# bertoldi-collab/DifFlexMM

Hardware: AMD Instinct MI355X
Metric: timesteps*rigid-units/s (forward + adjoint) (higher is better)
Workload: dtype f64

## Files before the change

difflexmm_amd/csrc/dfx_persist.h:

```cpp
#pragma once
#include "dfx_persist_api.h"

namespace {
using namespace dfx_persist;

typedef unsigned p_u4 __attribute__((ext_vector_type(4)));

__device__ __forceinline__ bool is_poison(double x) { return (unsigned)__double2hiint(x) == kPoisonWord; }

__device__ __forceinline__ void ring_load(const double* place, u32 byte_off, double (&r)[4]) {
  p_u4 c0, c1;
  asm volatile("global_load_dwordx4 %0, %2, %3 sc1\n\tglobal_load_dwordx4 %1, %2, %3 offset:16 sc1\n\ts_waitcnt vmcnt(0)"
               : "=&v"(c0), "=&v"(c1) : "v"(byte_off), "s"(place) : "memory");
  r[0] = __hiloint2double(c0.y, c0.x); r[1] = __hiloint2double(c0.w, c0.z);
  r[2] = __hiloint2double(c1.y, c1.x); r[3] = __hiloint2double(c1.w, c1.z);
}
__device__ __forceinline__ void ring_store(double* place, u32 byte_off, double a, double b) {
  p_u4 x;
  x.x = __double2loint(a); x.y = __double2hiint(a); x.z = __double2loint(b); x.w = __double2hiint(b);
  asm volatile("global_store_dwordx4 %0, %1, %2 sc1\n\ts_nop 1" ::"v"(byte_off), "v"(x), "s"(place) : "memory");
}
__device__ __forceinline__ void ring_poison(double* place, u32 byte_off) {
  p_u4 x; x.x = x.y = x.z = x.w = kPoisonWord;
  asm volatile("global_store_dwordx4 %0, %1, %2 sc1\n\ts_nop 1" ::"v"(byte_off), "v"(x), "s"(place) : "memory");
}

__global__ __launch_bounds__(kThreads) void k_ring_poison(double* ring, int batch, int n_blocks, int m0, int width , int places) {
  const int m = blockIdx.y + m0;
  const int tid = blockIdx.x * kThreads + threadIdx.x;
  if (tid >= n_blocks * width) return;
  const unsigned long long p = ~0ull;
  for (int pl = 0; pl < places; ++pl)
    reinterpret_cast<unsigned long long*>(ring)[((size_t)pl * batch + m) * ((size_t)n_blocks * width) + tid] = p;
}

struct LigRes {
  double rox, roy, rpx, rpy, lx, ly, l0, il0, ks, ksh, kr, sgn;
  double am, ac, kc, phi1, phi2, kap_safe, phi_min;
  int info, pslot;
};
template <int CONTACT>
__device__ __forceinline__ void load_lig_res(const DevCtx& c, const MemberBases& B, int slot, LigRes& g) {
  g.info = ldg<int>(c.slot_info, (u32)slot * 4);
  g.pslot = g.info < 0 ? slot : (g.info >> 1);
  g.sgn = (g.info & 1) ? 1.0 : -1.0;
  const double2 ro = ldg<double2>(B.p_r, (u32)slot * 16), rp = ldg<double2>(B.p_r, (u32)g.pslot * 16);
  g.rox = ro.x; g.roy = ro.y; g.rpx = rp.x; g.rpy = rp.y;
  if (c.l_dict_on) {
    const u32 li = (u32)ldg<uint8_t>(B.p_lidx, (u32)slot);
    const double2 lv = ldg<double2>(B.l_dict, li * 32), ln = ldg<double2>(B.l_dict, li * 32 + 16);
    g.lx = lv.x; g.ly = lv.y; g.l0 = ln.x; g.il0 = ln.y;
  } else {
    const double2 lv = ldg<double2>(B.p_l, (u32)slot * 16);
    g.lx = lv.x; g.ly = lv.y;
    g.l0 = g.info < 0 ? 1.0 : sqrt(lv.x * lv.x + lv.y * lv.y);
    g.il0 = 1.0 / g.l0;
  }
  if (c.k_uniform) { g.ks = B.cst[3]; g.ksh = B.cst[4]; g.kr = B.cst[5]; }
  else { g.ks = ldg<double>(B.p_k, (u32)slot * 32); g.ksh = ldg<double>(B.p_k, (u32)slot * 32 + 8); g.kr = ldg<double>(B.p_k, (u32)slot * 32 + 16); }
  g.am = g.ac = g.kc = g.phi1 = g.phi2 = g.kap_safe = g.phi_min = 0.0;
  if (CONTACT == 1) {
    g.am = B.cst[0]; g.ac = B.cst[1]; g.kc = B.cst[2]; g.kap_safe = B.cst[9]; g.phi_min = B.cst[10];
    const double2 ph = ldg<double2>(B.p_phi, (u32)slot * 16);
    g.phi1 = ph.x; g.phi2 = ph.y;
  }
}
__device__ __forceinline__ bool ring_wait(const double* place, u32 byte_off, double (&r)[4], int t_ord, int* give_up, int limit) {
  for (int spins = 0;;) {
    ring_load(place, byte_off, r);
    const bool ok = !(is_poison(r[0]) || is_poison(r[1]) || is_poison(r[2]) || is_poison(r[3]));
    if (__all(ok)) return true;
    if (++spins > limit) { *give_up = 1 + t_ord; return false; }
    __builtin_amdgcn_s_sleep(1);
  }
}

#ifdef DFX_PERSIST_TIMING
__device__ __forceinline__ unsigned long long tick() {
  unsigned long long t;
  asm volatile("s_waitcnt vmcnt(0) lgkmcnt(0)\n\ts_memtime %0\n\ts_waitcnt lgkmcnt(0)" : "=s"(t)::"memory");
  return t;
}
#if DFX_PERSIST_TIMING == 2
#define DFX_TICK(k) if ((k) < 4) { unsigned long long t_; asm volatile("s_memtime %0\n\ts_waitcnt lgkmcnt(0)" : "=s"(t_)::"memory"); acc_t[k] += (unsigned)(t_ - t_prev); t_prev = t_; }
#else
#define DFX_TICK(k) { const unsigned long long t_ = tick(); acc_t[k] += (unsigned)(t_ - t_prev); t_prev = t_; }
#endif
#else
#define DFX_TICK(k)
#endif

__device__ __forceinline__ bool persist_wave(const PersistArgs& pa, int& ml, int& w) {
  const int wv = (int)(threadIdx.x >> 6);
  if (pa.xcd_wg > 0) {
    const int xcd = (int)(blockIdx.x & 7), pos = (int)(blockIdx.x >> 3);
    const int mi = pos / pa.xcd_wg, j = pos - mi * pa.xcd_wg;
    ml = __builtin_amdgcn_readfirstlane(mi * 8 + xcd);
    w = __builtin_amdgcn_readfirstlane(j * (kPersistThreads / 64) + wv);
    return ml < pa.nm && w < pa.waves_per_member;
  }
  const int wave = __builtin_amdgcn_readfirstlane((int)(blockIdx.x * (kPersistThreads / 64)) + wv);
  if (wave >= pa.waves_per_member * pa.nm) return false;
  ml = wave / pa.waves_per_member;
  w = wave - ml * pa.waves_per_member;
  return true;
}

template <int NPB>
__device__ __forceinline__ LanePos wave_lane_pos(int w, int n_blocks) {
  LanePos p;
  const int gtid = w * 64 + (int)(threadIdx.x & 63);
  if (NPB == 4) { p.slot = gtid; p.b = gtid >> 2; p.k = gtid & 3; p.valid = p.b < n_blocks; return p; }
  const int j = gtid & 15;
  const int tri = min((j * 11) >> 5, 4);
  p.k = j - 3 * tri;
  p.b = (gtid >> 4) * 5 + tri;
  p.valid = p.b < n_blocks;
  p.slot = p.b * 4 + p.k;
  return p;
}

#ifndef DFX_PERSIST_OCC
#define DFX_PERSIST_OCC
#endif
template <int MODEL, int CONTACT, int NPB>
__global__ __launch_bounds__(kPersistThreads) DFX_PERSIST_OCC void k_fwd_persist(DevCtx c, PersistCoef pc, PersistArgs pa) {
  int ml, w;
  if (!persist_wave(pa, ml, w)) return;
  const int m = c.m0 + ml;
  const LanePos lp = wave_lane_pos<NPB>(w, c.n_blocks);
  if (!lp.valid) return;
  const int slot = lp.slot, b = lp.b, k = lp.k, kd = k < 3 ? k : 2;
  const u32 nd = (u32)c.n_blocks * 3;
  const int s = c.s;
  const Seg sg = *c.cur;
  const MemberBases B = member_bases(c, m);
  LigRes g;
  load_lig_res<CONTACT>(c, B, slot, g);
  const int info = g.info, pslot = g.pslot;
  const int dof = b * 3 + kd;
  const u32 o_dof = (u32)dof * 8, o_rec = ((u32)b * kPos + kd) * 8, o_chunk = ((u32)b * kPos + 2 * (k & 1)) * 8;
  const double damp = c.damping_uniform ? B.cst[6 + kd] : ldg<double>(c.damping + (size_t)((u32)m * nd), o_dof);
  const double invm = ldg<double>(c.inv_m + (size_t)((u32)m * nd), o_dof);
  const int sidx = ldg<int>(c.block_special, (u32)b * 4);
  const bool constrained = k < 3 && sidx >= 0 && ((c.special[sidx >= 0 ? sidx : 0].con_mask >> k) & 1);
  double tf_coef[DFX_MAX_FNS];
#pragma unroll
  for (int f = 0; f < DFX_MAX_FNS; ++f)
    tf_coef[f] = (k < 3 && sidx >= 0 && f < c.n_fns) ? (constrained ? c.special[sidx].con_coef[k][f] : c.special[sidx].load_coef[k][f]) : 0.0;
  const bool recs = c.rps > 1;
  const long long n0 = sg.base_step;
  double qn, vn;
  BlockRec<double> o;
  {
    const double* P0 = pos_in(c, m, recs ? -1 : 0, n0);
    const double* V0 = vel_in(c, m, recs ? -1 : 0, n0);
    const double2 a0 = ldg<double2>(P0, (u32)b * kPos * 8), a1 = ldg<double2>(P0, (u32)b * kPos * 8 + 16);
    o.x = a0.x; o.y = a0.y; o.th = a1.x; o.sh = a1.y;
    qn = ldg<double>(P0, o_rec);
    vn = ldg<double>(V0, o_dof);
  }
  double al[kPersistStages];
#pragma unroll
  for (int l = 0; l < kPersistStages; ++l) al[l] = 0.0;
  const size_t ring_stride = (size_t)c.batch * c.n_blocks * kPos;
  const u32 r_own = ((u32)m * (u32)c.n_blocks + (u32)b) * (kPos * 8) + 16u * (u32)(k & 1);
  const u32 r_par = ((u32)m * (u32)c.n_blocks + (u32)(pslot >> 2)) * (kPos * 8);
  if (k < 2) ring_store(pa.ring, r_own, k == 0 ? o.x : o.th, k == 0 ? o.y : o.sh);
  const int total = pa.n_steps * s;
  int t_ord = 0;
  double v_i = vn;
#ifdef DFX_PERSIST_TIMING
  unsigned acc_t[6] = {0, 0, 0, 0, 0, 0};
  unsigned long long t_prev = tick();
  const unsigned long long t_first = t_prev, w_first = wall_clock64();
#endif
  for (int j = 0; j < pa.n_steps; ++j) {
    const long long n = n0 + j;
    double h = sg.h;
    if (c.t_steps) { const double* ts = steps_of(c, m); h = ts[n + 1] - ts[n]; }
    double* Am = c.AD ? c.AD + (size_t)m * c.ad_stride + (size_t)n * ((u32)(s - 1) * nd) : nullptr;
#pragma unroll 1
    for (int i = 0; i < s; ++i) {
      {
        o.ch = half_cos(o.th, o.sh);
        double sv = 0.0, sq = 0.0, fload = 0.0;
#pragma unroll
        for (int l = 0; l < kPersistStages - 1; ++l) {
          const double a_l = l < i ? al[l] : 0.0;
          sv += pc.cv[i][l] * a_l;
          sq += pc.cq[i][l] * a_l;
        }
        double tv0[DFX_MAX_FNS], tv1[DFX_MAX_FNS];
#pragma unroll
        for (int f = 0; f < DFX_MAX_FNS; ++f) { tv0[f] = 0.0; tv1[f] = 0.0; }
        if (k < 3 && sidx >= 0) {
          const double* ft = fn_tab_row(c, m, j, constrained ? i + 1 : i);
          const u32 z = lane_zero();
#pragma unroll
          for (int f = 0; f < DFX_MAX_FNS; ++f)
            if (f < c.n_fns) { tv0[f] = fn_tab_get(ft, f, 0, z); if (constrained) tv1[f] = fn_tab_get(ft, f, 1, z); }
        }
        DFX_TICK(0)
        const double* place = pa.ring + (size_t)(t_ord % kPRing) * ring_stride;
        double pr[4];
        if (!ring_wait(place, r_par, pr, t_ord, pa.give_up, pa.spin_limit)) return;
        DFX_TICK(1)
        if (k < 2 && t_ord + kPAhead <= total) ring_poison(pa.ring + (size_t)((t_ord + kPAhead) % kPRing) * ring_stride, r_own);
        BlockRec<double> p;
        p.x = pr[0]; p.y = pr[1]; p.th = pr[2]; p.sh = pr[3];
        p.ch = half_cos(p.th, p.sh);
        double q_pre = 0.0, v_pre = 0.0;
#pragma unroll
        for (int f = 0; f < DFX_MAX_FNS; ++f) {
          if (constrained) { q_pre += tf_coef[f] * tv0[f]; v_pre += tf_coef[f] * tv1[f]; }
          else fload += tf_coef[f] * tv0[f];
        }
        double fx = 0.0, fy = 0.0, fth = 0.0;
        if (info >= 0) {
          BondGrad<double> bg;
          bond_grad<MODEL, double>(o, p, g.rox, g.roy, g.rpx, g.rpy, g.lx, g.ly, g.l0, g.il0, g.ks, g.ksh, g.kr, g.sgn, bg);
          fx = bg.fx; fy = bg.fy; fth = bg.fth;
          if (CONTACT == 1) {
            const bool far = !(fabs(o.th - p.th) <= g.kap_safe);
            ContactGrad<double> cg;
            contact_grad<double>(g.sgn * (o.th - p.th), far ? g.phi1 : g.phi_min, far ? g.phi2 : g.phi_min, g.am, g.ac, g.kc, cg);
            fth += g.sgn * cg.dkap;
          }
        }
        DFX_TICK(2)
        const double dE = blk_reduce3<NPB>(fx, fy, fth, k);
        double qnext = 0.0, vnext = 0.0;
        if (k < 3) {
          const double a = constrained ? 0.0 : (fload - dE - damp * v_i) * invm;
          if (Am && i < s - 1) stg<double>(Am + (size_t)i * nd, o_dof, a);
          sv += pc.cv[i][i] * a;
          sq += pc.cq[i][i] * a;
#pragma unroll
          for (int l = 0; l < kPersistStages; ++l) al[l] = l == i ? a : al[l];
          qnext = qn + h * (pc.c[i + 1] * vn + h * sq);
          vnext = vn + h * sv;
          if (constrained) { qnext = q_pre; vnext = v_pre; }
        }
        DFX_TICK(3)
        const double y1 = blk_bcast<NPB, 1>(qnext, k), th2 = blk_bcast<NPB, 2>(qnext, k), x0 = blk_bcast<NPB, 0>(qnext, k);
        double sn, cs;
        fast_sincos(0.5 * th2, &sn, &cs);
        o.x = x0; o.y = y1; o.th = th2; o.sh = sn;
        ++t_ord;
        DFX_TICK(4)
        const bool last = i == s - 1;
        if (k < 2) ring_store(pa.ring + (size_t)(t_ord % kPRing) * ring_stride, r_own, k == 0 ? x0 : th2, k == 0 ? y1 : sn);
        if (k < 3) {
          const double2 chunk = k == 0 ? make_double2(x0, y1) : make_double2(th2, sn);
          if (recs || (last && c.traj)) {
            double* tr = recs ? traj_rec(c, m, -2 - i, n) : traj_rec(c, m, -1, n + 1);
            if (k < 2) stg<double2>(tr, o_chunk, chunk);
            stg<double>(tr + (size_t)c.n_blocks * kPos, o_dof, vnext);
          }
          if (last && !recs && j == pa.n_steps - 1) {
            if (k < 2) stg<double2>(c.POS + (size_t)((u32)m * (u32)c.nbuf * (u32)c.n_blocks * kPos), o_chunk, chunk);
            stg<double>(c.VEL + (size_t)((u32)m * (u32)c.nbuf * nd), o_dof, vnext);
          }
        }
        v_i = vnext;
        if (last) { qn = qnext; vn = vnext; }
        DFX_TICK(5)
      }
    }
  }
#ifdef DFX_PERSIST_TIMING
  if (pa.dbg && (threadIdx.x & 63) == 0) {
    unsigned* d = pa.dbg + (size_t)(blockIdx.x * 4 + (threadIdx.x >> 6)) * 8;
    for (int q = 0; q < 6; ++q) d[q] = acc_t[q];
    d[6] = (unsigned)(tick() - t_first); d[7] = (unsigned)total;
  }
  if (blockIdx.x == 0 && threadIdx.x == 0) {
    for (int q = 0; q < 6; ++q) pa.give_up[1 + q] = (int)acc_t[q];
    pa.give_up[7] = (int)(tick() - t_first);
    pa.give_up[8] = (int)(wall_clock64() - w_first);
    pa.give_up[9] = total;
  }
#endif
}



template <int MODEL, int CONTACT, int NPB, int DENSE>
__device__ __forceinline__ void adj_persist_body(const DevCtx& c, const PersistAdjCoef& pc, const PersistArgs& pa, const DenseCtx& dn) {
  int ml, w;
  if (!persist_wave(pa, ml, w)) return;
  const int m = c.m0 + ml;
  const LanePos lp = wave_lane_pos<NPB>(w, c.n_blocks);
  if (!lp.valid) return;
  const int slot = lp.slot, b = lp.b, k = lp.k, kd = k < 3 ? k : 2;
  const u32 nd = (u32)c.n_blocks * 3, nd6 = (u32)c.n_blocks * 6;
  const int s = c.s;
  const Seg sg = *c.cur;
  long long n_m = 0;
  int j_top = pa.n_steps - 1;
  if constexpr (DENSE) {
    n_m = dn.n_acc[m];
    if (n_m - sg.base_step < (long long)j_top) j_top = (int)(n_m - sg.base_step);
    if (j_top < 0) return;
  }
  const MemberBases B = member_bases(c, m);
  LigRes g;
  load_lig_res<CONTACT>(c, B, slot, g);
  const int info = g.info, pslot = g.pslot;
  const int dof = b * 3 + kd;
  const u32 o_dof = (u32)dof * 8, o_b6 = ((u32)b * 6 + 2 * kd) * 8;
  const double damp = c.damping_uniform ? B.cst[6 + kd] : ldg<double>(c.damping + (size_t)((u32)m * nd), o_dof);
  const double invm = ldg<double>(c.inv_m + (size_t)((u32)m * nd), o_dof);
  const int sidx = ldg<int>(c.block_special, (u32)b * 4);
  const bool constrained = k < 3 && sidx >= 0 && ((c.special[sidx >= 0 ? sidx : 0].con_mask >> k) & 1);
  double tf_coef[DFX_MAX_FNS];
#pragma unroll
  for (int f = 0; f < DFX_MAX_FNS; ++f)
    tf_coef[f] = (k < 3 && sidx >= 0 && f < c.n_fns) ? (constrained ? c.special[sidx].con_coef[k][f] : c.special[sidx].load_coef[k][f]) : 0.0;
  double* LAMm = c.LAM + (size_t)((u32)m * nd6);
  const u32 ms = (u32)m * (u32)c.n_slots;
  double* grm = c.g_r + (size_t)(ms * 2);
  double* gpm = c.g_phi + (size_t)ms;
  double* bmm = c.blk_m + (size_t)((u32)m * nd);
  double* bcm = c.blk_c ? c.blk_c + (size_t)((u32)m * nd) : nullptr;
  __shared__ double2 s_yb[kPersistStages - 1][kPersistThreads];
  __shared__ double2 s_racc[kPersistThreads];
  __shared__ double s_acc[3][kPersistThreads];
  __shared__ double2 s_lam[kPersistThreads];
  const int tid = (int)threadIdx.x;
  s_racc[tid] = ldg<double2>(grm, (u32)slot * 16);
  s_lam[tid] = ldg<double2>(LAMm, o_b6);
  s_acc[0][tid] = CONTACT == 1 ? ldg<double>(gpm, (u32)slot * 8) : 0.0;
  s_acc[1][tid] = ldg<double>(bmm, o_dof);
  s_acc[2][tid] = bcm ? ldg<double>(bcm, o_dof) : 0.0;
  bool phi_any = false;
  const size_t ring_stride = (size_t)c.batch * c.n_blocks * kPos;
  const u32 r_own = ((u32)m * (u32)c.n_blocks + (u32)b) * (kPos * 8) + 16u * (u32)(k & 1);
  const u32 r_par = ((u32)m * (u32)c.n_blocks + (u32)(pslot >> 2)) * (kPos * 8);
  const int total = DENSE ? (j_top + 1) * s - ((sg.base_step + j_top == n_m) ? s - 1 : 0) : pa.n_steps * s;
  int t_ord = 0;
#ifdef DFX_PERSIST_TIMING
  unsigned acc_t[6] = {0, 0, 0, 0, 0, 0};
  unsigned long long t_prev = tick();
  const unsigned long long t_first = t_prev;
#endif
  for (int j = j_top; j >= 0; --j) {
    const long long n = sg.base_step + j;
    double h = sg.h, h_before = (sg.j0 + j) == 0 ? sg.h_prev : sg.h;
    if (c.t_steps) { const double* ts = steps_of(c, m); h = ts[n + 1] - ts[n]; h_before = n > 0 ? ts[n] - ts[n - 1] : 0.0; }
#pragma unroll 1
    for (int i = (DENSE && n == n_m) ? 0 : s - 1; i >= 0; --i) {
      const int win = (int)((n * s + i) & 1);
      const double* POSin = traj_rec(c, m, -1 - i, n);
      const double2 o0 = ldg<double2>(POSin, (u32)b * (kPos * 8)), o1 = ldg<double2>(POSin, (u32)b * (kPos * 8) + 16);
      const double2 q0 = ldg<double2>(POSin, (u32)(pslot >> 2) * (kPos * 8)), q1 = ldg<double2>(POSin, (u32)(pslot >> 2) * (kPos * 8) + 16);
      const double v_i = ldg<double>(POSin + (size_t)c.n_blocks * kPos, o_dof);
      double sq = 0.0, sv = 0.0, sqc = 0.0, svc = 0.0;
#pragma unroll
      for (int jj = 1; jj < kPersistStages; ++jj) {
        const bool on = jj > i && jj < s && !(DENSE && n == n_m);
        const double2 y = on ? s_yb[jj - 1][tid] : make_double2(0.0, 0.0);
        const double cf = i > 0 ? pc.col[i][jj] : 1.0;
        sq += cf * y.x;
        sv += cf * y.y;
        sqc += pc.cur[i][jj] * y.x;
        svc += pc.cur[i][jj] * y.y;
      }
      double tv0[DFX_MAX_FNS];
#pragma unroll
      for (int f = 0; f < DFX_MAX_FNS; ++f) tv0[f] = 0.0;
      if (k < 3 && sidx >= 0 && !constrained) {
        const double* ft = fn_tab_row(c, m, j, i);
        const u32 z = lane_zero();
#pragma unroll
        for (int f = 0; f < DFX_MAX_FNS; ++f) if (f < c.n_fns) tv0[f] = fn_tab_get(ft, f, 0, z);
      }
      const double col_s = pc.col[i][s], cur_s = pc.cur[i][s], col_i = pc.col[i][i];
      const double2 lam = s_lam[tid];
      const double lq = lam.x, lv = lam.y;
      double w_d = (h * (cur_s * lv + svc)) * invm;
      double e_own_q = 0.0, e_nxt_v = 0.0, gs_q = 0.0, gs_v = 0.0;
      if constexpr (DENSE) {
        if (!constrained) {
          const int* op = dn.out_ptr + (size_t)m * dn.stride;
          const int lo = op[n], hi = op[n + 1], plo = n > 0 ? op[n - 1] : lo;
          const double* dwm = dn.dw + (size_t)m * dn.n_out * 8;
          const u32 o_g = ((u32)b * 6 + kd) * 8;
          double e_own_v = 0.0;
          for (int kk = lo; kk < hi; ++kk) {
            const double* Gk = c.G + ((size_t)kk * c.batch + m) * (size_t)nd6;
            const double gq = ldg<double>(Gk, o_g), gv = ldg<double>(Gk, o_g + 24);
            const double* wt = dwm + (size_t)kk * 8;
            e_own_q += wt[i] * gq; e_own_v += wt[i] * gv;
            if (i > 0) e_nxt_v += wt[i - 1] * gv;
            else { gs_q += gq; gs_v += gv; }
          }
          e_own_q *= h; e_own_v *= h; e_nxt_v *= h;
          if (i <= 1) {
            double e6q = 0.0, e6v = 0.0, e5v = 0.0;
            for (int kk = plo; kk < lo; ++kk) {
              const double* Gk = c.G + ((size_t)kk * c.batch + m) * (size_t)nd6;
              const double gq = ldg<double>(Gk, o_g), gv = ldg<double>(Gk, o_g + 24);
              const double* wt = dwm + (size_t)kk * 8;
              e6q += wt[6] * gq; e6v += wt[6] * gv;
              e5v += wt[s - 1] * gv;
            }
            if (i == 0) { e_own_q += h_before * e6q; e_own_v += h_before * e6v; e_nxt_v = h_before * e5v; }
            else e_nxt_v += h_before * e6v;
          }
          if (i == 0 && n == 0)
            for (int kk = 0; kk < lo; ++kk) {
              const double* Gk = c.G + ((size_t)kk * c.batch + m) * (size_t)nd6;
              gs_q += ldg<double>(Gk, o_g); gs_v += ldg<double>(Gk, o_g + 24);
            }
          w_d += e_own_v * invm;
        }
      }
      const double wox = blk_bcast<NPB, 0>(w_d, k), woy = blk_bcast<NPB, 1>(w_d, k), woth = blk_bcast<NPB, 2>(w_d, k);
      double wp[4];
      DFX_TICK(0)
      if (t_ord == 0) {
        const double* Win = c.W + (size_t)(((u32)m * 2 + (u32)win) * nd);
        const u32 pb = (u32)(pslot >> 2) * 24;
        const double2 wxy = ldg<double2>(Win, pb);
        wp[0] = wxy.x; wp[1] = wxy.y; wp[2] = ldg<double>(Win, pb + 16);
      } else if (!ring_wait(pa.ring + (size_t)(t_ord % kPRing) * ring_stride, r_par, wp, t_ord, pa.give_up, pa.spin_limit)) return;
      DFX_TICK(1)
      if (k < 2 && t_ord + kPAhead < total) ring_poison(pa.ring + (size_t)((t_ord + kPAhead) % kPRing) * ring_stride, r_own);
      BlockRec<double> o, p;
      o.x = o0.x; o.y = o0.y; o.th = o1.x; o.sh = o1.y; o.ch = half_cos(o.th, o.sh);
      p.x = q0.x; p.y = q0.y; p.th = q1.x; p.sh = q1.y; p.ch = half_cos(p.th, p.sh);
      double hx = 0.0, hy = 0.0, hth = 0.0, ex = 0.0, ey = 0.0, eth = 0.0, d_rx = 0.0, d_ry = 0.0, d_phi = 0.0;
      if (info >= 0) {
        BondHvp hv;
        bond_hvp<MODEL>(o, p, wox, woy, woth, wp[0], wp[1], wp[2], g.rox, g.roy, g.rpx, g.rpy, g.lx, g.ly, g.l0, g.il0, g.ks, g.ksh, g.kr, g.sgn, hv);
        hx = hv.hx; hy = hv.hy; hth = hv.hth;
        ex = hv.fx; ey = hv.fy; eth = hv.fth;
        d_rx = hv.rx; d_ry = hv.ry;
        if (CONTACT == 1) {
          const bool far = !(fabs(o.th - p.th) <= g.kap_safe);
          double dk, dke, p1e, p2e;
          contact_hvp(g.sgn * (o.th - p.th), g.sgn * (woth - wp[2]), far ? g.phi1 : g.phi_min, far ? g.phi2 : g.phi_min, g.am, g.ac, g.kc, dk, dke, p1e, p2e);
          hth += g.sgn * dke;
          eth += g.sgn * dk;
          d_phi = (info & 1) ? p2e : p1e;
        }
        const double2 r_old = s_racc[tid];
        s_racc[tid] = make_double2(r_old.x - d_rx, r_old.y - d_ry);
      }
      if (CONTACT == 1 && d_phi != 0.0) { s_acc[0][tid] -= d_phi; phi_any = true; }
      DFX_TICK(2)
      const double hw = blk_reduce3<NPB>(hx, hy, hth, k);
      const double dE = blk_reduce3<NPB>(ex, ey, eth, k);
      double w_next = 0.0;
      if (k < 3) {
        double fload = 0.0;
#pragma unroll
        for (int f = 0; f < DFX_MAX_FNS; ++f) if (!constrained) fload += tf_coef[f] * tv0[f];
        if (c.fn_g && sidx >= 0) {
          const double* ft = fn_tab_row(c, m, j, i);
#pragma unroll
          for (int f = 0; f < DFX_MAX_FNS; ++f) {
            const double coef = f < c.n_fns ? (constrained ? -hw * tf_coef[f] : w_d * tf_coef[f]) : 0.0;
            if (coef != 0.0) {
              const u32 z = lane_zero();
              double* q = c.fn_g + (((size_t)m * c.n_special + sidx) * DFX_MAX_FNS + f) * DFX_FN_PARAMS;
              for (int kk = 0; kk < DFX_FN_PARAMS; ++kk) acc_add(q + kk, coef * fn_tab_get(ft, f, 2 + kk, z));
            }
          }
        }
        const double a_i = constrained ? 0.0 : (fload - dE - damp * v_i) * invm;
        double kq_in = h * (cur_s * lq + sqc);
        if constexpr (DENSE) kq_in += e_own_q;
        double ybq = 0.0, ybv = 0.0;
        if (!constrained) {
          ybq = -hw;
          ybv = kq_in - damp * w_d;
          s_acc[1][tid] -= w_d * a_i;
          s_acc[2][tid] -= w_d * v_i;
        }
        if (i > 0) s_yb[i - 1][tid] = make_double2(ybq, ybv);
        double kv;
        if (i > 0) {
          kv = h * (col_s * lv + col_i * ybv + sv);
        } else {
          double nlq = lq + (ybq + sq), nlv = lv + (ybv + sv);
          if constexpr (DENSE) { nlq += gs_q; nlv += gs_v; }
          const bool first = !DENSE && (sg.j0 + j) == 0;
          if (first && c.G && !constrained) {
            const double* G = c.G + ((size_t)sg.interval * c.batch + m) * (size_t)nd6;
            nlq += G[b * 6 + k]; nlv += G[b * 6 + 3 + k];
          }
          if (constrained) { nlq = 0.0; nlv = 0.0; }
          s_lam[tid] = make_double2(nlq, nlv);
          kv = h_before * col_s * nlv;
        }
        if constexpr (DENSE) kv += e_nxt_v;
        w_next = constrained ? 0.0 : kv * invm;
      }
      DFX_TICK(3)
      ++t_ord;
      if (t_ord < total) {
        const double w1 = blk_bcast<NPB, 1>(w_next, k), w2 = blk_bcast<NPB, 2>(w_next, k);
        if (k < 2) ring_store(pa.ring + (size_t)(t_ord % kPRing) * ring_stride, r_own, k == 0 ? w_next : w2, k == 0 ? w1 : 0.0);
      } else if (k < 3) {
        stg<double>(c.W + (size_t)(((u32)m * 2 + (u32)(win ^ 1)) * nd), o_dof, w_next);
      }
    }
  }
#ifdef DFX_PERSIST_TIMING
  if (pa.dbg && (threadIdx.x & 63) == 0) {
    unsigned* d = pa.dbg + (size_t)(blockIdx.x * 4 + (threadIdx.x >> 6)) * 8;
    for (int q = 0; q < 6; ++q) d[q] = acc_t[q];
    d[6] = (unsigned)(tick() - t_first); d[7] = (unsigned)total;
  }
#endif
  if (info >= 0) stg<double2>(grm, (u32)slot * 16, s_racc[tid]);
  if (CONTACT == 1 && phi_any) { stg<double>(gpm, (u32)slot * 8, s_acc[0][tid]); c.touch[0] = 1; }
  if (k < 3) {
    stg<double2>(LAMm, o_b6, s_lam[tid]);
    if (!constrained) { stg<double>(bmm, o_dof, s_acc[1][tid]); if (bcm) stg<double>(bcm, o_dof, s_acc[2][tid]); }
  }
}

template <int MODEL, int CONTACT, int NPB>
__global__ __launch_bounds__(kPersistThreads) __attribute__((amdgpu_waves_per_eu(3))) void k_adj_persist(DevCtx c, PersistAdjCoef pc, PersistArgs pa) {
  adj_persist_body<MODEL, CONTACT, NPB, 0>(c, pc, pa, DenseCtx{});
}

}
```

difflexmm_amd/csrc/dfx_persist_api.h:

```cpp
#pragma once
#include <hip/hip_runtime.h>

namespace dfx_persist {

constexpr int kPRing = 8;
constexpr int kPAhead = 4;
constexpr int kPersistThreads = 256;
constexpr unsigned kPoisonWord = 0xFFFFFFFFu;
constexpr int kPersistStages = 6;
constexpr int kSpinLimit = 1 << 23;
static_assert(kPAhead >= 2 && kPRing >= kPAhead + 1, "hand-off ring: re-poison at least two ordinals ahead, ring longer than the look-ahead");

struct PersistCoef {
  double cv[kPersistStages][kPersistStages];
  double cq[kPersistStages][kPersistStages];
  double c[kPersistStages + 1];
};
struct PersistArgs {
  double* ring;
  int* give_up;
  int n_steps, nm, waves_per_member;
  int spin_limit;
  int xcd_wg;
#ifdef DFX_PERSIST_TIMING
  unsigned* dbg;
#endif
};


struct PersistAdjCoef {
  double col[kPersistStages][kPersistStages + 1];
  double cur[kPersistStages][kPersistStages + 1];
  double c[kPersistStages];
};

const void* fwd_kernel(int model, int contact, int npb);
const void* adj_kernel(int model, int contact, int npb);
const void* adaptive_fwd_kernel(int model, int contact);
const void* adj_dense_kernel(int model, int contact, int npb);
void launch_ring_poison(hipStream_t st, double* ring, int batch, int n_blocks, int m0, int nm, int width);

}
```

difflexmm_amd/csrc/dfx_persist_dense.h:

```cpp
#pragma once
#include "dfx_persist.h"
#include "dfx_dense.h"

template <int CTRL> __device__ __forceinline__ double dpp_row_mov(double v) {
  int lo = __double2loint(v), hi = __double2hiint(v);
  lo = __builtin_amdgcn_update_dpp(lo, lo, CTRL, 0xf, 0xf, false);
  hi = __builtin_amdgcn_update_dpp(hi, hi, CTRL, 0xf, 0xf, false);
  return __hiloint2double(hi, lo);
}
__device__ __forceinline__ double lanes_plus_32(double v) {
  const unsigned lo = (unsigned)__double2loint(v), hi = (unsigned)__double2hiint(v);
  const auto a = __builtin_amdgcn_permlane32_swap(lo, lo, false, false);
  const auto b = __builtin_amdgcn_permlane32_swap(hi, hi, false, false);
  return __hiloint2double((int)b[1], (int)a[1]);
}
__device__ __forceinline__ double lanes_plus_16(double v) {
  const unsigned lo = (unsigned)__double2loint(v), hi = (unsigned)__double2hiint(v);
  const auto a = __builtin_amdgcn_permlane16_swap(lo, lo, false, false);
  const auto b = __builtin_amdgcn_permlane16_swap(hi, hi, false, false);
  return __hiloint2double((int)b[1], (int)a[1]);
}
__device__ __forceinline__ double wave_sum_lane0(double v) {
  v += lanes_plus_32(v);
  v += lanes_plus_16(v);
  v += dpp_row_mov<0x108>(v);
  v += dpp_row_mov<0x104>(v);
  v += dpp_row_mov<0x102>(v);
  v += dpp_row_mov<0x101>(v);
  return v;
}
__device__ __forceinline__ double lane_value(double v, int lane_uniform) {
  return __hiloint2double(__builtin_amdgcn_readlane(__double2hiint(v), lane_uniform), __builtin_amdgcn_readlane(__double2loint(v), lane_uniform));
}

#ifndef DFX_DENSE_OCC
#define DFX_DENSE_OCC __attribute__((amdgpu_waves_per_eu(3)))
#endif
namespace {

__device__ __forceinline__ double err_load(const double* p) {
  double v;
  asm volatile("global_load_dwordx2 %0, %1, off sc1\n\ts_waitcnt vmcnt(0)" : "=&v"(v) : "v"(p) : "memory");
  return v;
}
__device__ __forceinline__ void err_store(double* p, double v) {
  asm volatile("global_store_dwordx2 %0, %1, off sc1\n\ts_nop 1" ::"v"(p), "v"(v) : "memory");
}

template <int MODEL, int CONTACT>
__global__ __launch_bounds__(kPersistThreads) void k_adaptive_fwd_loop(DevCtx c, AdaptLoopCoef pc, PersistArgs pa, AdaptLoopArgs aa) {
  int ml, w;
  if (!persist_wave(pa, ml, w)) return;
  const int W = pa.waves_per_member;
  const int m = c.m0 + ml;
  Clock ck = c.clock[m];
  if (ck.state) return;
  LanePos lp = wave_lane_pos<4>(w, c.n_blocks);
  const bool valid = lp.valid;
  if (!valid) { lp.b = c.n_blocks - 1; lp.k = (int)(threadIdx.x & 3); lp.slot = lp.b * 4 + lp.k; }
  const int slot = lp.slot, b = lp.b, k = lp.k, kd = k < 3 ? k : 2;
  const int lane = (int)(threadIdx.x & 63);
  const u32 nd = (u32)c.n_blocks * 3;
  const MemberBases B = member_bases(c, m);
  LigRes g;
  load_lig_res<CONTACT>(c, B, slot, g);
  const int info = g.info, pslot = g.pslot;
  const int dof = b * 3 + kd;
  const u32 o_dof = (u32)dof * 8, o_rec = ((u32)b * kPos + kd) * 8, o_chunk = ((u32)b * kPos + 2 * (k & 1)) * 8;
  const double damp = c.damping_uniform ? B.cst[6 + kd] : ldg<double>(c.damping + (size_t)((u32)m * nd), o_dof);
  const double invm = ldg<double>(c.inv_m + (size_t)((u32)m * nd), o_dof);
  const int sidx = ldg<int>(c.block_special, (u32)b * 4);
  const bool constrained = k < 3 && sidx >= 0 && ((c.special[sidx >= 0 ? sidx : 0].con_mask >> k) & 1);
  const bool dof_lane = valid && k < 3;
  const bool keep = aa.keep != 0;
  double tf_coef[DFX_MAX_FNS];
#pragma unroll
  for (int f = 0; f < DFX_MAX_FNS; ++f)
    tf_coef[f] = (valid && k < 3 && sidx >= 0 && f < c.n_fns) ? (constrained ? c.special[sidx].con_coef[k][f] : c.special[sidx].load_coef[k][f]) : 0.0;
  double* Am = c.A + (size_t)((u32)m * (u32)(c.s + 1) * nd);
  long long n_acc = ck.accepted;
  double qn, vn;
  BlockRec<double> o;
  {
    const double* P0 = pos_in(c, m, keep ? -1 : 0, n_acc);
    const double* V0 = vel_in(c, m, keep ? -1 : 0, n_acc);
    const double2 a0 = ldg<double2>(P0, (u32)b * kPos * 8), a1 = ldg<double2>(P0, (u32)b * kPos * 8 + 16);
    o.x = a0.x; o.y = a0.y; o.th = a1.x; o.sh = a1.y;
    qn = ldg<double>(P0, o_rec);
    vn = ldg<double>(V0, o_dof);
  }
  double al[7];
  al[0] = ldg<double>(Am, o_dof);
#pragma unroll
  for (int l = 1; l < 7; ++l) al[l] = 0.0;
  const size_t ring_stride = (size_t)c.batch * c.n_blocks * kPos;
  const u32 r_own = ((u32)m * (u32)c.n_blocks + (u32)b) * (kPos * 8) + 16u * (u32)(k & 1);
  const u32 r_par = ((u32)m * (u32)c.n_blocks + (u32)(pslot >> 2)) * (kPos * 8);
  const size_t err_stride = (size_t)c.batch * W;
  double* err_m = aa.err + (size_t)m * W;
  const double* ts_out = c.ts_dev;
  const int Tn = aa.n_timepoints;
  double t = ck.t, h = ck.h;
  double t_out_next = ck.out_idx < Tn ? ts_out[ck.out_idx] : 1.7976931348623157e308;
  int t_ord = 0;
  long long attempt = 0;
  for (; attempt < pa.n_steps; ++attempt) {
    if (keep && n_acc + 3 > aa.cap) break;
    double fg[DFX_MAX_FNS], fgt[DFX_MAX_FNS];
    const bool need_fn = c.n_fns > 0 && __any(sidx >= 0);
    if (need_fn) {
      const int jj = min(lane & 7, 6);
      const double cj = jj == 0 ? pc.c[0] : (jj == 1 ? pc.c[1] : (jj == 2 ? pc.c[2] : (jj == 3 ? pc.c[3] : (jj == 4 ? pc.c[4] : (jj == 5 ? pc.c[5] : pc.c[6])))));
      double gp[kMaxFnParams];
#pragma unroll
      for (int f = 0; f < DFX_MAX_FNS; ++f) {
        fg[f] = 0.0; fgt[f] = 0.0;
        if (f < c.n_fns) eval_time_fn(c.fns[(u32)m * DFX_MAX_FNS + f], t + cj * h, fg[f], fgt[f], gp);
      }
    }
    auto prescribed = [&](int j, double& q, double& v) {
      if (!need_fn) return;
      double sq_ = 0.0, sv_ = 0.0;
#pragma unroll
      for (int f = 0; f < DFX_MAX_FNS; ++f) {
        const double gj = lane_value(fg[f], j), gtj = lane_value(fgt[f], j);
        if (constrained && f < c.n_fns) { sq_ += tf_coef[f] * gj; sv_ += tf_coef[f] * gtj; }
      }
      if (constrained) { q = sq_; v = sv_; }
    };
    auto load_at = [&](int j) -> double {
      double fl = 0.0;
      if (!need_fn) return fl;
#pragma unroll
      for (int f = 0; f < DFX_MAX_FNS; ++f) {
        const double gj = lane_value(fg[f], j);
        if (k < 3 && sidx >= 0 && !constrained && f < c.n_fns) fl += tf_coef[f] * gj;
      }
      return fl;
    };
    double v_i;
    {
      double qx = qn + h * pc.a[1][0] * vn, vx = vn + h * pc.a[1][0] * al[0];
      prescribed(1, qx, vx);
      v_i = vx;
      const double y1 = blk_bcast<4, 1>(qx, k), th2 = blk_bcast<4, 2>(qx, k), x0 = blk_bcast<4, 0>(qx, k);
      double sn, cs;
      fast_sincos(0.5 * th2, &sn, &cs);
      o.x = x0; o.y = y1; o.th = th2; o.sh = sn;
      if (valid && k < 2) ring_store(pa.ring + (size_t)(t_ord % kPRing) * ring_stride, r_own, k == 0 ? x0 : th2, k == 0 ? y1 : sn);
      if (keep && dof_lane) {
        double* tr = traj_rec(c, m, -2, n_acc);
        if (k < 2) stg<double2>(tr, o_chunk, k == 0 ? make_double2(x0, y1) : make_double2(th2, sn));
        stg<double>(tr + (size_t)c.n_blocks * kPos, o_dof, vx);
      }
    }
    double q1 = 0.0, v1 = 0.0, r2 = 0.0;
#pragma unroll 1
    for (int i = 1; i <= 6; ++i) {
      o.ch = half_cos(o.th, o.sh);
      double sv = 0.0, sq = 0.0, fload = 0.0;
#pragma unroll
      for (int l = 0; l < 6; ++l) {
        const double a_l = l < i ? al[l] : 0.0;
        sv += (i < 6 ? pc.a[i + 1][l] : pc.e[l]) * a_l;
        sq += (i < 6 ? pc.aa[i + 1][l] : pc.ee[l]) * a_l;
      }
      fload = load_at(i);
      double pr[4];
      if (!ring_wait(pa.ring + (size_t)(t_ord % kPRing) * ring_stride, r_par, pr, t_ord, pa.give_up, pa.spin_limit)) return;
      if (valid && k < 2) ring_poison(pa.ring + (size_t)((t_ord + kPAhead) % kPRing) * ring_stride, r_own);
      BlockRec<double> p;
      p.x = pr[0]; p.y = pr[1]; p.th = pr[2]; p.sh = pr[3];
      p.ch = half_cos(p.th, p.sh);
      double fx = 0.0, fy = 0.0, fth = 0.0;
      if (info >= 0) {
        BondGrad<double> bg;
        bond_grad<MODEL, double>(o, p, g.rox, g.roy, g.rpx, g.rpy, g.lx, g.ly, g.l0, g.il0, g.ks, g.ksh, g.kr, g.sgn, bg);
        fx = bg.fx; fy = bg.fy; fth = bg.fth;
        if (CONTACT == 1) {
          const bool far = !(fabs(o.th - p.th) <= g.kap_safe);
          ContactGrad<double> cg;
          contact_grad<double>(g.sgn * (o.th - p.th), far ? g.phi1 : g.phi_min, far ? g.phi2 : g.phi_min, g.am, g.ac, g.kc, cg);
          fth += g.sgn * cg.dkap;
        }
      }
      const double dE = blk_reduce3<4>(fx, fy, fth, k);
      const double a = constrained ? 0.0 : (fload - dE - damp * v_i) * invm;
      ++t_ord;
      if (i < 6) {
        sv += pc.a[i + 1][i] * a;
        sq += pc.aa[i + 1][i] * a;
#pragma unroll
        for (int l = 1; l < 7; ++l) al[l] = l == i ? a : al[l];
        double qx = qn + h * (pc.c[i + 1] * vn + h * sq), vx = vn + h * sv;
        prescribed(i + 1, qx, vx);
        const double y1 = blk_bcast<4, 1>(qx, k), th2 = blk_bcast<4, 2>(qx, k), x0 = blk_bcast<4, 0>(qx, k);
        double sn, cs;
        fast_sincos(0.5 * th2, &sn, &cs);
        o.x = x0; o.y = y1; o.th = th2; o.sh = sn;
        if (valid && k < 2) ring_store(pa.ring + (size_t)(t_ord % kPRing) * ring_stride, r_own, k == 0 ? x0 : th2, k == 0 ? y1 : sn);
        if (keep && dof_lane) {
          double* tr = traj_rec(c, m, -2 - i, n_acc);
          if (k < 2) stg<double2>(tr, o_chunk, k == 0 ? make_double2(x0, y1) : make_double2(th2, sn));
          stg<double>(tr + (size_t)c.n_blocks * kPos, o_dof, vx);
        }
        v_i = vx;
        if (i == 5) { q1 = qx; v1 = vx; }
      } else {
        al[6] = a;
        sv += pc.e[6] * a;
        sq += pc.ee[6] * a;
        if (dof_lane && !constrained) {
          const double eq = h * h * sq, ev = h * sv;
          const double tq = c.atol + c.rtol * fmax(fabs(qn), fabs(q1)), tv = c.atol + c.rtol * fmax(fabs(vn), fabs(v1));
          r2 = (eq / tq) * (eq / tq) + (ev / tv) * (ev / tv);
        }
      }
    }
    r2 = wave_sum_lane0(r2);
    double* slot_now = err_m + (size_t)(attempt % 3) * err_stride;
    if (lane == 0) err_store(slot_now + w, r2);
    double acc_a = 0.0, acc_b = 0.0;
    for (int r = 0; r * 64 < W; ++r) {
      const int idx = lane + 64 * r;
      double v = 0.0;
      if (idx < W) {
        for (int spins = 0;;) {
          v = err_load(slot_now + idx);
          if (!is_poison(v)) break;
          if (++spins > pa.spin_limit) { *pa.give_up = -1 - (int)(attempt & 0xffff); return; }
          __builtin_amdgcn_s_sleep(1);
        }
      }
      if (r & 1) acc_b += v; else acc_a += v;
    }
    if (lane == 0) err_store(err_m + (size_t)((attempt + 2) % 3) * err_stride + w, __hiloint2double((int)kPoisonWord, (int)kPoisonWord));
    double red = acc_a + acc_b;
    red = lane_value(wave_sum_lane0(red), 0);
    const double ratio = sqrt(red / aa.two_n_free);
    ck.attempts++;
    if (!(ratio == ratio)) { ck.state = 2; break; }
    const double h_new = dopri_next_step(h, ratio);
    if (ratio <= 1.0) {
      const double t_new = t + h;
      const int out_lo = ck.out_idx;
      int out_hi = out_lo;
      if (t_out_next <= t_new) {
        while (out_hi < Tn && ts_out[out_hi] <= t_new) ++out_hi;
        t_out_next = out_hi < Tn ? ts_out[out_hi] : 1.7976931348623157e308;
      }
      if (dof_lane && out_hi > out_lo) {
        double sm = pc.cm[0] * al[0] + pc.cm[6] * al[6], sma = pc.cma[0] * al[0] + pc.cma[6] * al[6];
#pragma unroll
        for (int l = 1; l < 6; ++l) { sm += pc.cm[l] * al[l]; sma += pc.cma[l] * al[l]; }
        const double qmid = qn + h * (0.5 * vn + h * sma), vmid = vn + h * sm;
        for (int kk = out_lo; kk < out_hi; ++kk) {
          const double tk = ts_out[kk];
          const double r = (tk - t) / (t_new - t);
          double oq = dopri_dense(qn, q1, qmid, vn, v1, h, r), ov = dopri_dense(vn, v1, vmid, al[0], al[6], h, r);
          if (constrained) { const TimeVals tv = constrained_value(c, m, c.special[sidx], k, tk); oq = tv.g; ov = tv.gt; }
          double* f = c.fields_dev + ((size_t)m * Tn + kk) * c.n_blocks * 6;
          stg<double>(f, o_dof, oq);
          stg<double>(f + nd, o_dof, ov);
        }
      }
      if (w == 0 && lane == 0) {
        if (c.acc_times && n_acc + 1 <= c.acc_cap) c.acc_times[(size_t)m * c.acc_cap + n_acc] = t_new;
        if (c.step_counts && Tn > 1) c.step_counts[(size_t)m * (Tn - 1) + min(max(out_lo - 1, 0), Tn - 2)]++;
        if (aa.ar.t_steps) {
          double* ts = aa.ar.t_steps + (size_t)m * aa.ar.stride;
          int* op = aa.ar.out_ptr + (size_t)m * aa.ar.stride;
          ts[n_acc + 1] = t_new; ts[n_acc + 2] = t_new;
          op[n_acc] = out_lo; op[n_acc + 1] = out_hi; op[n_acc + 2] = out_hi;
          for (int kk = out_lo; kk < out_hi; ++kk) aa.ar.theta[(size_t)m * Tn + kk] = (ts_out[kk] - t) / (t_new - t);
        }
      }
      ck.t_last = t; ck.h_acc = h; ck.out_lo = out_lo; ck.out_hi = out_hi; ck.out_idx = out_hi; ck.accepted++;
      t = t_new; ++n_acc;
      qn = q1; vn = v1; al[0] = al[6];
      if (out_hi >= Tn) { ck.state = 1; ck.h = h_new; break; }
    }
    ck.accept = ratio <= 1.0;
    h = h_new;
    if (!(h > 0.0)) { ck.state = 3; break; }
  }
  ck.t = t; if (ck.state != 1) ck.h = h;
  if (w == 0 && lane == 0) c.clock[m] = ck;
  const double y1 = blk_bcast<4, 1>(qn, k), th2 = blk_bcast<4, 2>(qn, k), x0 = blk_bcast<4, 0>(qn, k);
  double sn, cs;
  fast_sincos(0.5 * th2, &sn, &cs);
  if (dof_lane) {
    stg<double>(Am, o_dof, al[0]);
    if (!keep) {
      if (k < 2) stg<double2>(c.POS + (size_t)((u32)m * (u32)c.nbuf * (u32)c.n_blocks * kPos), o_chunk, k == 0 ? make_double2(x0, y1) : make_double2(th2, sn));
      stg<double>(c.VEL + (size_t)((u32)m * (u32)c.nbuf * nd), o_dof, vn);
    }
  }
}

template <int MODEL, int CONTACT, int NPB>
__global__ __launch_bounds__(kPersistThreads) DFX_DENSE_OCC void k_adj_dense_loop(DevCtx c, PersistAdjCoef pc, PersistArgs pa,
                                                                                                           DenseCtx dn) {
  adj_persist_body<MODEL, CONTACT, NPB, 1>(c, pc, pa, dn);
}

}
```

difflexmm_amd/csrc/engine_launch.hip:

```cpp
#include "dfx_engine.h"
#include <climits>

using namespace dfx_persist;

void drop_graphs(dfx_handle* h) {
  for (auto& kv : h->graphs) (void)hipGraphExecDestroy(kv.second);
  h->graphs.clear();
  h->graph_ctx_valid = false;
  if (h->adaptive_exec) { (void)hipGraphExecDestroy(h->adaptive_exec); h->adaptive_exec = nullptr; }
}

DevCtx make_ctx(dfx_handle* h) {
  const Plan& pl = h->pl;
  DevCtx c;
  memset(&c, 0, sizeof(c));
  c.n_blocks = pl.n_blocks; c.n_slots = pl.n_slots; c.n_fns = pl.n_fns; c.batch = pl.batch; c.s = pl.tab.s;
#ifdef DFX_ABLATE
  { const char* a = getenv("DFX_ABLATE"); c.ablate = a ? atoi(a) : 0; }
#endif
  c.n_wg = (pl.n_slots + kThreads - 1) / kThreads;
  c.n_wg3 = (pl.n_blocks + (kThreads / 16) * 5 - 1) / ((kThreads / 16) * 5);
  for (int k = 0; k < 4; ++k) c.pred[k] = pl.pred_delta[k];
  c.nbuf = 2 * pl.tab.s;
  c.n_special = pl.n_special; c.k_uniform = h->pp.k_uniform ? 1 : 0; c.n_timepoints = (int)h->ts.size();
  c.slot_info = h->d_slot_info.p; c.block_special = h->d_block_special.p; c.special = h->d_special.p;
  c.n_ovf = pl.n_ovf;
  if (pl.n_ovf) { c.ovf_ptr = h->d_ovf_ptr.p; c.ovf_info = h->d_ovf_info.p; c.ovf_p = h->d_ovf_p.p; c.ovf_g = h->d_ovf_g.p; }
  c.p_lidx = h->d_l_idx.p; c.l_dict = h->d_l_dict.p; c.l_dict_on = h->pp.l_dict_ok ? 1 : 0; c.damping_uniform = h->pp.damping_uniform ? 1 : 0;
  { const char* e = getenv("DFX_DICT_LDS"); c.l_dict_lds = (h->pp.l_dict_ok && h->pp.n_dict_max <= kDictLds && !(e && e[0] == '0')) ? 1 : 0; }
  c.p_r = h->d_p_r.p; c.p_l = h->d_p_l.p; c.p_k = h->d_p_k.p; c.p_phi = h->d_p_phi.p; c.cst = h->d_cst.p;
  c.inv_m = h->d_inv_m.p; c.damping = h->d_damping.p; c.fns = h->d_fns.p;
  c.p_c = h->d_p_c.p; c.g_c = h->d_g_c.p; c.n_npb = pl.n_npb;
  c.cur = h->d_cur.p;
  c.fn_tab = nullptr;
  c.clock = h->adaptive ? h->d_clock.p : nullptr;
  c.err_partial = h->d_err_partial.p; c.ts_dev = h->d_ts.p; c.fields_dev = h->d_fields.p;
  c.step_counts = h->adaptive ? h->d_step_counts.p : nullptr;
  c.acc_times = h->adaptive ? h->d_acc_times.p : nullptr; c.acc_cap = kAccCap;
  c.t_steps = (!h->adaptive && !h->t_steps.empty()) ? h->d_tsteps.p : nullptr;
  c.ts_stride = c.t_steps ? h->ts_stride : 0;
  c.rtol = h->rtol; c.atol = h->atol;
  c.traj = h->have_traj ? h->ck->traj.p : nullptr;
  c.rps = (h->have_traj && (h->records || h->segments)) ? pl.tab.s : 1;
  c.AD = (h->have_traj && h->dense && !h->records && !h->segments) ? h->ck->AD.p : nullptr;
  c.ad_stride = pl.batch ? (long long)(h->ck->AD.n / pl.batch) : 0;
  c.POS = h->d_POS.p; c.VEL = h->d_VEL.p; c.A = h->d_A.p;
  c.YB = h->d_YB.p; c.LAM = h->d_LAM.p; c.W = h->d_W.p; c.KQ = h->d_KQ.p; c.G = h->d_G.p;
  c.g_r = h->d_g_r.p; c.g_phi = h->d_g_phi.p; c.g_b = (h->want_bond_grads || pl.n_ovf) ? h->d_g_b.p : nullptr;
  c.touch = h->d_touch.p;
  c.lam_pairs = (c.g_b || c.AD) ? 0 : 1;
  c.blk_m = h->d_blk_m.p; c.blk_c = h->want_damping_grads ? h->d_blk_c.p : nullptr;
  c.fn_g = h->want_fn_grads ? h->d_fn_g.p : nullptr;
  return c;
}

dim3 slot_grid(const dfx_handle* h) { return dim3((h->pl.n_slots + kThreads - 1) / kThreads, h->pl.batch); }
dim3 slot_grid(const dfx_handle* h, const Group& g) { return dim3((h->pl.n_slots + kThreads - 1) / kThreads, g.nm); }
DevCtx group_ctx(const dfx_handle* h, const DevCtx& c, int gi) {
  DevCtx cg = c;
  cg.m0 = h->groups[gi].m0;
  cg.cur = h->d_cur.p + gi;
  return cg;
}

StageCoef stage_coef(const Tableau& T, int i) {
  StageCoef sc;
  memset(&sc, 0, sizeof(sc));
  const int r = i + 1;
  for (int l = 0; l <= i; ++l) { sc.cv[l] = T.a[r][l]; sc.cq[l] = T.aa[r][l]; }
  sc.c_i = T.c[i];
  sc.c_next = T.c[r];
  return sc;
}
AdjCoef adj_coef(const Tableau& T, int i) {
  AdjCoef ac;
  memset(&ac, 0, sizeof(ac));
  if (i > 0) {
    for (int j = i; j < T.s; ++j) ac.col[j] = T.a[j][i - 1];
    ac.col[T.s] = T.a[T.s][i - 1];
  } else {
    ac.col[T.s] = T.a[T.s][T.s - 1];
  }
  for (int j = i + 1; j < T.s; ++j) ac.cur[j] = T.a[j][i];
  ac.cur[T.s] = T.a[T.s][i];
  ac.c_i = T.c[i];
  return ac;
}

#ifdef DFX_EXPERIMENTAL
#include "dfx_experimental_host.h"
#else
void setup_tiling(dfx_handle*) {}
void setup_lig(dfx_handle*) {}
int lig_pack(dfx_handle*) { return 0; }
void pair_plan(dfx_handle* h, const DevCtx&) { h->pair_fwd = h->pair_adj = false; }
bool lig_fwd_ok(const dfx_handle*, const DevCtx&, int) { return false; }
bool lig_adj_ok(const dfx_handle*, const DevCtx&, int, int) { return false; }
#endif
int pair_state_buf(const dfx_handle* h, long long n) {
#ifdef DFX_EXPERIMENTAL
  if (h->pair_fwd) return state_buf(n);
#endif
  (void)h; (void)n;
  return 0;
}

bool pack3(const dfx_handle* h) {
  const char* e = getenv("DFX_PACK3");
  return h->pl.n_npb == 3 && !h->adaptive && !(e && e[0] == '0');
}
static bool hot_shape(const DevCtx& c) {
  return c.k_uniform && c.l_dict_on && c.l_dict_lds && c.damping_uniform && !c.t_steps && !c.AD && !c.clock;
}
template <int MODEL, int CONTACT, int NPB>
static bool launch_fwd_hot(dfx_handle* h, const DevCtx& c, hipStream_t st, dim3 grid, int i, int j, int in_buf, int out_buf, int y_buf, int mode) {
  if constexpr ((MODEL == kNonlinear || MODEL == kLinearized) && CONTACT != 2) {
    if (!h->wt || !h->stage_builds || !hot_shape(c)) return false;
    const StageCoef scf = stage_coef(h->pl.tab, i);
    const bool recs = c.rps > 1 && in_buf == -1 - i && out_buf == -2 - i && y_buf == -1 && mode == 0;
#define DFX_FWD_I(I)                                                                                                              \
  case I:                                                                                                                         \
    if (recs)                                                                                                                     \
      hipLaunchKernelGGL((k_fwd_stage<MODEL, CONTACT, NPB, 1, 0, 1, I, 1>), grid, dim3(kThreads), 0, st, c, scf, i, j, in_buf, out_buf, \
                         y_buf, mode);                                                                                            \
    else                                                                                                                          \
      hipLaunchKernelGGL((k_fwd_stage<MODEL, CONTACT, NPB, 1, 0, 1, I, 0>), grid, dim3(kThreads), 0, st, c, scf, i, j, in_buf, out_buf, \
                         y_buf, mode);                                                                                            \
    return true;
    switch (i) { DFX_FWD_I(0) DFX_FWD_I(1) DFX_FWD_I(2) DFX_FWD_I(3) DFX_FWD_I(4) DFX_FWD_I(5) default: break; }
#undef DFX_FWD_I
  }
  return false;
}
namespace dfx_hot {
bool launch_adj_stage_build(int model, int contact, int npb, hipStream_t st, dim3 grid, const DevCtx& c, const AdjCoef& acf, int i, int j, int in_buf, int wbuf,
                            int local_only, const StageCoef& rc, int rb);
}
template <int MODEL, int CONTACT, int NPB>
static bool launch_adj_hot(dfx_handle* h, const DevCtx& c, hipStream_t st, dim3 grid, int i, int j, int in_buf, int wbuf, int local_only, const StageCoef& rc,
    int rb) {
  if constexpr ((MODEL == kNonlinear || MODEL == kLinearized) && CONTACT != 2) {
    if (!h->wt || !h->stage_builds || !(c.k_uniform && c.l_dict_on && c.l_dict_lds && c.damping_uniform && !c.t_steps)) return false;
    return dfx_hot::launch_adj_stage_build(MODEL, CONTACT, NPB, st, grid, c, adj_coef(h->pl.tab, i), i, j, in_buf, wbuf, local_only, rc, rb);
  }
  return false;
}
int kernel_build_code(const dfx_handle* h, const DevCtx& c, bool tile) {
  if (tile) return 1;
  const bool model_ok = (h->pl.model == kNonlinear || h->pl.model == kLinearized) && h->pl.contact != DFX_CONTACT_DISTANCE;
  const bool quad_or_packed = !h->pl.n_ovf && (h->pl.n_npb == 4 || pack3(h));
  return (model_ok && quad_or_packed && h->wt && h->stage_builds && c.fn_tab && hot_shape(c) && h->pl.tab.s <= 6) ? 2 : 0;
}
template <int MODEL, int CONTACT>
static void launch_fwd_t(dfx_handle* h, const DevCtx& c, hipStream_t st, dim3 grid, int i, int j, int in_buf, int out_buf, int y_buf, int mode) {
#ifdef DFX_EXPERIMENTAL
  if constexpr (CONTACT != 2) {
    if (lig_fwd_ok(h, c, mode)) {
      const dim3 tg(h->lig.n_wg, grid.y);
      hipLaunchKernelGGL((k_fwd_tile<MODEL, CONTACT>), tg, dim3(64 * kTileWaves), 0, st, c, h->lig, stage_coef(h->pl.tab, i), i, j, in_buf, out_buf,
                         y_buf, mode);
      return;
    }
  }
#endif
  if (h->pl.n_ovf) {
    if constexpr (CONTACT != 2)
      hipLaunchKernelGGL((k_fwd_stage<MODEL, CONTACT, 4, 0, 1>), grid, dim3(kThreads), 0, st, c, stage_coef(h->pl.tab, i), i, j, in_buf, out_buf, y_buf, mode);
    return;
  }
  const bool tab = c.fn_tab != nullptr && !c.clock;
  if (CONTACT != 2 && pack3(h) && !(mode & 2)) {
    if constexpr (CONTACT != 2) {
      if (tab && launch_fwd_hot<MODEL, CONTACT, 3>(h, c, st, dim3(c.n_wg3, grid.y), i, j, in_buf, out_buf, y_buf, mode)) return;
      if (tab) hipLaunchKernelGGL((k_fwd_stage<MODEL, CONTACT, 3, 1>), dim3(c.n_wg3, grid.y), dim3(kThreads), 0, st, c, stage_coef(h->pl.tab, i), i, j,
          in_buf, out_buf, y_buf, mode);
      else hipLaunchKernelGGL((k_fwd_stage<MODEL, CONTACT, 3, 0>), dim3(c.n_wg3, grid.y), dim3(kThreads), 0, st, c, stage_coef(h->pl.tab, i), i, j, in_buf,
          out_buf, y_buf, mode);
    }
    return;
  }
  if (tab && h->wt) {
    if (launch_fwd_hot<MODEL, CONTACT, 4>(h, c, st, grid, i, j, in_buf, out_buf, y_buf, mode)) return;
    hipLaunchKernelGGL((k_fwd_stage<MODEL, CONTACT, 4, 1, 0, 1>), grid, dim3(kThreads), 0, st, c, stage_coef(h->pl.tab, i), i, j, in_buf, out_buf, y_buf, mode);
  }
  else if (tab) hipLaunchKernelGGL((k_fwd_stage<MODEL, CONTACT, 4, 1>), grid, dim3(kThreads), 0, st, c, stage_coef(h->pl.tab, i), i, j, in_buf, out_buf,
      y_buf, mode);
  else hipLaunchKernelGGL((k_fwd_stage<MODEL, CONTACT, 4, 0>), grid, dim3(kThreads), 0, st, c, stage_coef(h->pl.tab, i), i, j, in_buf, out_buf, y_buf, mode);
}
void launch_fwd(dfx_handle* h, const DevCtx& c, hipStream_t st, dim3 grid, int i, int j, int in_buf, int out_buf, int y_buf, int mode) {
  const Plan& pl = h->pl;
#define DFX_FWD_CASE(M) case M: if (pl.contact == 2) launch_fwd_t<M, 2>(h, c, st, grid, i, j, in_buf, out_buf, y_buf, mode); \
    else if (pl.contact) launch_fwd_t<M, 1>(h, c, st, grid, i, j, in_buf, out_buf, y_buf, mode); else launch_fwd_t<M, 0>(h, c, st, grid, i, j, in_buf, \
    out_buf, y_buf, mode); break;
  switch (pl.model) { DFX_FWD_CASE(kNonlinear) DFX_FWD_CASE(kLinearized) DFX_FWD_CASE(kSimpleSpring) DFX_FWD_CASE(kStretchTorsion) }
#undef DFX_FWD_CASE
  h->launches++;
}
void launch_fwd(dfx_handle* h, const DevCtx& c, int i, int j, int in_buf, int out_buf, int y_buf, int mode) {
  launch_fwd(h, c, h->stream, slot_grid(h), i, j, in_buf, out_buf, y_buf, mode);
}
template <int MODEL, int CONTACT>
static void launch_adj_t(dfx_handle* h, const DevCtx& c, hipStream_t st, dim3 grid, int i, int j, int in_buf, int wbuf, int local_only) {
  const int s = h->pl.tab.s;
  const int rb = (c.AD && !local_only) ? (i >= 2 ? i - 1 : (i == 0 ? s - 1 : 0)) : 0;
  const StageCoef rc = stage_coef(h->pl.tab, rb > 0 ? rb - 1 : 0);
#ifdef DFX_EXPERIMENTAL
  if constexpr (CONTACT != 2) {
    if (lig_adj_ok(h, c, wbuf, local_only)) {
      const dim3 tg(h->lig.n_wg, grid.y);
      hipLaunchKernelGGL((k_adj_tile<MODEL, CONTACT>), tg, dim3(64 * kTileWaves), 0, st, c, h->lig, adj_coef(h->pl.tab, i), i, j, in_buf);
      return;
    }
  }
#endif
  if (h->pl.n_ovf) {
    if constexpr (CONTACT != 2)
      hipLaunchKernelGGL((k_adj_stage<MODEL, CONTACT, 1, 1, 4, 0, 1>), grid, dim3(kThreads), 0, st, c, adj_coef(h->pl.tab, i), i, j, in_buf, wbuf, local_only,
          rc, rb);
  }
  else if (c.g_b) hipLaunchKernelGGL((k_adj_stage<MODEL, CONTACT, 1, 1>), grid, dim3(kThreads), 0, st, c, adj_coef(h->pl.tab, i), i, j, in_buf, wbuf,
      local_only, rc, rb);
  else if (c.AD) hipLaunchKernelGGL((k_adj_stage_rb<MODEL, CONTACT>), grid, dim3(kThreads), 0, st, c, adj_coef(h->pl.tab, i), i, j, in_buf, wbuf, local_only,
      rc, rb);
  else if (CONTACT != 2 && pack3(h)) {
    if constexpr (CONTACT != 2) {
      if (c.fn_tab && !local_only && launch_adj_hot<MODEL, CONTACT, 3>(h, c, st, dim3(c.n_wg3, grid.y), i, j, in_buf, wbuf, local_only, rc, rb)) return;
      if (c.fn_tab && !local_only) hipLaunchKernelGGL((k_adj_stage<MODEL, CONTACT, 0, 0, 3, 1>), dim3(c.n_wg3, grid.y), dim3(kThreads), 0, st, c,
          adj_coef(h->pl.tab, i), i, j, in_buf, wbuf, local_only, rc, rb);
      else hipLaunchKernelGGL((k_adj_stage<MODEL, CONTACT, 0, 0, 3, 0>), dim3(c.n_wg3, grid.y), dim3(kThreads), 0, st, c, adj_coef(h->pl.tab, i), i, j,
          in_buf, wbuf, local_only, rc, rb);
    }
  }
  else if (c.fn_tab && !local_only && h->wt) {
    if (launch_adj_hot<MODEL, CONTACT, 4>(h, c, st, grid, i, j, in_buf, wbuf, local_only, rc, rb)) return;
    hipLaunchKernelGGL((k_adj_stage<MODEL, CONTACT, 0, 0, 4, 1, 0, 1>), grid, dim3(kThreads), 0, st, c, adj_coef(h->pl.tab, i), i, j, in_buf, wbuf,
        local_only, rc, rb);
  }
  else if (c.fn_tab && !local_only) hipLaunchKernelGGL((k_adj_stage<MODEL, CONTACT, 0, 0, 4, 1>), grid, dim3(kThreads), 0, st, c, adj_coef(h->pl.tab, i), i,
      j, in_buf, wbuf, local_only, rc, rb);
  else hipLaunchKernelGGL((k_adj_stage<MODEL, CONTACT, 0, 0, 4, 0>), grid, dim3(kThreads), 0, st, c, adj_coef(h->pl.tab, i), i, j, in_buf, wbuf, local_only,
      rc, rb);
}
void launch_adj(dfx_handle* h, const DevCtx& c, hipStream_t st, dim3 grid, int i, int j, int in_buf, int wbuf, int local_only) {
  const Plan& pl = h->pl;
#define DFX_ADJ_CASE(M) case M: if (pl.contact == 2) launch_adj_t<M, 2>(h, c, st, grid, i, j, in_buf, wbuf, local_only); \
    else if (pl.contact) launch_adj_t<M, 1>(h, c, st, grid, i, j, in_buf, wbuf, local_only); else launch_adj_t<M, 0>(h, c, st, grid, i, j, in_buf, wbuf, \
    local_only); break;
  switch (pl.model) { DFX_ADJ_CASE(kNonlinear) DFX_ADJ_CASE(kLinearized) DFX_ADJ_CASE(kSimpleSpring) DFX_ADJ_CASE(kStretchTorsion) }
#undef DFX_ADJ_CASE
  h->launches++;
}
void launch_adj(dfx_handle* h, const DevCtx& c, int i, int j, int in_buf, int wbuf, int local_only) {
  launch_adj(h, c, h->stream, slot_grid(h), i, j, in_buf, wbuf, local_only);
}

static const int kPersistSlots = 64;
struct PersistInflight { hipEvent_t ev; hipStream_t st; int slots; };
static std::mutex g_persist_mu;
static std::vector<PersistInflight> g_persist_inflight[64];
static std::vector<hipEvent_t> g_persist_events[64];

static int persist_wg_slots(const void* fn) {
  static std::mutex mu;
  static std::map<const void*, int> cache;
  std::lock_guard<std::mutex> lk(mu);
  auto it = cache.find(fn);
  if (it != cache.end()) return it->second;
  hipFuncAttributes at;
  if (!fn || hipFuncGetAttributes(&at, fn) != hipSuccess) { (void)hipGetLastError(); return 0; }
  const int alloc = std::max(8, ((at.numRegs + 7) / 8) * 8);
  return cache[fn] = alloc > 512 ? 0 : alloc / 8;
}
static int persist_wg_per_cu(const void* fn) {
  static std::mutex mu;
  static std::map<const void*, int> cache;
  std::lock_guard<std::mutex> lk(mu);
  auto it = cache.find(fn);
  if (it != cache.end()) return it->second;
  int nb = 0;
  if (!fn || hipOccupancyMaxActiveBlocksPerMultiprocessor(&nb, fn, kPersistThreads, 0) != hipSuccess) { (void)hipGetLastError(); nb = 0; }
  return cache[fn] = nb;
}
bool persist_shape_ok(const dfx_handle* h) {
  const Plan& pl = h->pl;
  const char* e = getenv("DFX_PERSIST");
  if ((e && e[0] == '0') || h->persist_off) return false;
  return (pl.model == kNonlinear || pl.model == kLinearized) && pl.contact != DFX_CONTACT_DISTANCE && !pl.n_ovf && pl.tab.s <= kPersistStages &&
         (pl.n_npb == 3 || pl.n_npb == 4);
}
static int persist_waves_per_member(const dfx_handle* h, int npb) {
  return npb == 3 ? (h->pl.n_blocks + 19) / 20 : (h->pl.n_slots + 63) / 64;
}
static int persist_cap(const void* fn);
int persist_members_that_fit(dfx_handle* h, const void* fn, int npb) {
  if (!h->n_cu) { int v = 0; if (hipDeviceGetAttribute(&v, hipDeviceAttributeMultiprocessorCount, h->device) != hipSuccess || v <= 0) return 0; h->n_cu = v; }
  const int cap = persist_cap(fn);
  const long long wpm = persist_waves_per_member(h, npb);
  if (cap <= 0 || wpm <= 0) return 0;
  return (int)std::min<long long>(h->pl.batch, ((long long)cap * h->n_cu * 4) / wpm);
}
static int persist_cap(const void* fn) {
  const int wg_slots = persist_wg_slots(fn);
  int cap = wg_slots ? std::min(8, kPersistSlots / wg_slots) : 0;
  if (const int occ = persist_wg_per_cu(fn)) cap = std::min(cap, occ);
  if (const char* e = getenv("DFX_PERSIST_MAX_WG")) cap = std::min(cap, atoi(e));
  return cap;
}
static void persist_shape(const dfx_handle* h, int npb, int nm, int* grid, int* per_cu, const void* fn = nullptr, int* xcd_wg = nullptr) {
  const long long wpm = persist_waves_per_member(h, npb);
  if (xcd_wg) {
    *xcd_wg = 0;
    const char* e = getenv("DFX_PERSIST_XCD");
    const int wg = (int)((wpm + 3) / 4), cus = h->n_cu / 8, per_xcd = (nm + 7) / 8, cap = fn ? persist_cap(fn) : 0;
    if (!(e && e[0] == '0') && h->n_cu % 8 == 0 && wg <= cus && (long long)per_xcd * wg <= (long long)cap * cus) {
      *xcd_wg = wg;
      *grid = 8 * per_xcd * wg;
      *per_cu = std::max(1, (per_xcd * wg + cus - 1) / cus);
      return;
    }
  }
  const long long waves = (long long)nm * wpm;
  const long long g = (waves + 3) / 4;
  *grid = (int)g;
  *per_cu = (int)std::max<long long>(1, (g + h->n_cu - 1) / h->n_cu);
}
static int persist_max_chunks() {
  const char* e = getenv("DFX_PERSIST_CHUNKS");
  return e ? std::max(1, atoi(e)) : 2;
}
static int persist_adj_max_chunks() {
  const char* e = getenv("DFX_PERSIST_ADJ_CHUNKS");
  return e ? std::max(1, atoi(e)) : INT_MAX;
}
static int chunk_members(int nm, int n_chunks, int k) { return nm / n_chunks + (k < nm % n_chunks ? 1 : 0); }
static bool persist_common_ok(dfx_handle* h, const DevCtx& c, bool any_groups = false) {
  if (!persist_shape_ok(h) || h->adaptive || (h->groups.size() != 1 && !any_groups)) return false;
  if (h->pl.n_fns > 0 && !c.fn_tab) return false;
  h->persist_npb = (h->pl.n_npb == 3 && pack3(h)) ? 3 : 4;
  h->persist_wpm = persist_waves_per_member(h, h->persist_npb);
  return true;
}
bool persist_members_ok(const dfx_handle* h, int per_launch) {
  return per_launch > 0 && (h->pl.batch + per_launch - 1) / per_launch <= persist_max_chunks();
}
static bool persist_adj_members_ok(const dfx_handle* h, const void* fn, int per_launch) {
  if (persist_members_ok(h, per_launch)) return true;
  const int nm = h->pl.batch, n_chunks = per_launch > 0 ? (nm + per_launch - 1) / per_launch : 0;
  if (n_chunks <= 0 || n_chunks > persist_adj_max_chunks()) return false;
  const long long room = (long long)persist_cap(fn) * h->n_cu * 4;
  return 2LL * chunk_members(nm, n_chunks, n_chunks - 1) * h->persist_wpm >= room;
}
bool persist_would_serve(dfx_handle* h) {
  if (!persist_shape_ok(h) || h->adaptive || h->groups.size() != 1) return false;
  const int npb = (h->pl.n_npb == 3 && pack3(h)) ? 3 : 4;
  return persist_members_ok(h, persist_members_that_fit(h, dfx_persist::fwd_kernel(h->pl.model, h->pl.contact, npb), npb)) &&
         persist_members_ok(h, persist_members_that_fit(h, dfx_persist::adj_kernel(h->pl.model, h->pl.contact, npb), npb));
}
void persist_plan(dfx_handle* h, const DevCtx& c) {
  h->persist_fwd = false;
  if (h->pair_fwd || h->lig_fwd_used || !persist_common_ok(h, c)) return;
  const void* fn = dfx_persist::fwd_kernel(h->pl.model, h->pl.contact, h->persist_npb);
  if (!fn) return;
  h->persist_fwd_members = persist_members_that_fit(h, fn, h->persist_npb);
  if (!persist_members_ok(h, h->persist_fwd_members)) return;
  if (h->d_ring.ensure((size_t)kPRing * h->pl.batch * h->pl.n_blocks * kPos) != hipSuccess) { (void)hipGetLastError(); return; }
  h->persist_fwd = true;
}
void persist_plan_adj(dfx_handle* h, const DevCtx& c) {
  h->persist_adj = false;
  const bool wide = h->records;
  if (h->pair_adj || h->lig_adj_used || !persist_common_ok(h, c, wide)) return;
  if (c.rps <= 1 || c.g_b || c.AD || !c.lam_pairs) return;
  const void* fn = dfx_persist::adj_kernel(h->pl.model, h->pl.contact, h->persist_npb);
  if (!fn) return;
  h->persist_adj_members = persist_members_that_fit(h, fn, h->persist_npb);
  if (!(wide ? persist_adj_members_ok(h, fn, h->persist_adj_members) : persist_members_ok(h, h->persist_adj_members))) return;
  if (h->d_ring.ensure((size_t)kPRing * h->pl.batch * h->pl.n_blocks * kPos) != hipSuccess) { (void)hipGetLastError(); return; }
  h->persist_adj = true;
}
static PersistCoef persist_coef(const Tableau& T) {
  PersistCoef pc;
  memset(&pc, 0, sizeof(pc));
  for (int i = 0; i < T.s && i < kPersistStages; ++i)
    for (int l = 0; l <= i; ++l) { pc.cv[i][l] = T.a[i + 1][l]; pc.cq[i][l] = T.aa[i + 1][l]; }
  for (int r = 0; r <= T.s && r <= kPersistStages; ++r) pc.c[r] = T.c[r];
  return pc;
}
int* persist_give_up_word(dfx_handle* h) { return reinterpret_cast<int*>(h->flag_stage.p) + 2; }
int ensure_flags(dfx_handle* h) {
  HIP_OK(h->flag_stage.ensure(64 + sizeof(int) * (size_t)h->pl.batch));
  return 0;
}
int* member_flags(dfx_handle* h) { return reinterpret_cast<int*>(h->flag_stage.p) + 16; }
#ifdef DFX_PERSIST_TIMING
unsigned* persist_dbg_buffer() { static unsigned* p = nullptr; if (!p) { (void)hipHostMalloc((void**)&p, 8 * 4 * 8192 * sizeof(unsigned), hipHostMallocDefault); memset(p, 0, 8 * 4 * 8192 * sizeof(unsigned)); } return p; }
#endif
int persist_spin_limit(const dfx_handle* h) { return h->spin_limit > 0 ? h->spin_limit : kSpinLimit; }
void persist_fell_back(dfx_handle* h) {
  h->persist_off = true;
  h->persist_fwd = h->persist_adj = false;
  static bool said = false;
  if (!said) fprintf(stderr, "[dfx] a persistent launch could not get all its workgroups resident (another process on the device?): this engine keeps one "
                             "launch per stage from now on; the solve is run again that way\n");
  said = true;
}
void persist_forget(dfx_handle* h) {
  std::lock_guard<std::mutex> lk(g_persist_mu);
  auto& fl = g_persist_inflight[h->device & 63];
  for (size_t i = 0; i < fl.size();) {
    bool mine = fl[i].st == h->stream;
    for (auto& g : h->groups) mine = mine || fl[i].st == g.stream || fl[i].st == g.stream2;
    if (mine) { (void)hipEventSynchronize(fl[i].ev); g_persist_events[h->device & 63].push_back(fl[i].ev); fl.erase(fl.begin() + i); } else ++i;
  }
}
static void launch_persist(dfx_handle* h, const void* fn, hipStream_t st, void** args, int grid, int need) {
  std::lock_guard<std::mutex> lk(g_persist_mu);
  const int d = h->device & 63;
  auto& fl = g_persist_inflight[d];
  for (size_t i = 0; i < fl.size();)
    if (hipEventQuery(fl[i].ev) == hipSuccess) { g_persist_events[d].push_back(fl[i].ev); fl.erase(fl.begin() + i); } else { (void)hipGetLastError(); ++i; }
  for (;;) {
    std::map<hipStream_t, std::pair<int, size_t>> other;
    for (size_t i = 0; i < fl.size(); ++i)
      if (fl[i].st != st) { auto& o = other[fl[i].st]; o.first = std::max(o.first, fl[i].slots); o.second = i; }
    int total = need;
    for (auto& kv : other) total += kv.second.first;
    if (total <= kPersistSlots || other.empty()) break;
    auto victim = other.begin();
    for (auto it = other.begin(); it != other.end(); ++it) if (it->second.second < victim->second.second) victim = it;
    (void)hipStreamWaitEvent(st, fl[victim->second.second].ev, 0);
    const hipStream_t vs = victim->first;
    for (size_t i = 0; i < fl.size();)
      if (fl[i].st == vs) { fl[i].st = st; ++i; } else ++i;
  }
  (void)hipLaunchKernel(fn, dim3(grid), dim3(kPersistThreads), args, 0, st);
  hipEvent_t ev = nullptr;
  if (!g_persist_events[d].empty()) { ev = g_persist_events[d].back(); g_persist_events[d].pop_back(); }
  else (void)hipEventCreateWithFlags(&ev, hipEventDisableTiming);
  (void)hipEventRecord(ev, st);
  fl.push_back({ev, st, need});
  h->launches++;
}
static void launch_segment_persist(dfx_handle* h, const DevCtx& c, hipStream_t st, int nm, int n_steps, bool reverse, double* ring = nullptr) {
  if (!ring) ring = h->d_ring.p;
  const int npb = h->persist_npb, per = reverse ? h->persist_adj_members : h->persist_fwd_members;
  const void* fn = reverse ? dfx_persist::adj_kernel(h->pl.model, h->pl.contact, npb) : dfx_persist::fwd_kernel(h->pl.model, h->pl.contact, npb);
  PersistCoef pcf = persist_coef(h->pl.tab);
  PersistAdjCoef pca;
  memset(&pca, 0, sizeof(pca));
  for (int i = 0; i < h->pl.tab.s && i < kPersistStages; ++i) {
    const AdjCoef ac = adj_coef(h->pl.tab, i);
    for (int jj = 0; jj <= kPersistStages; ++jj) { pca.col[i][jj] = ac.col[jj]; pca.cur[i][jj] = ac.cur[jj]; }
    pca.c[i] = ac.c_i;
  }
  const int n_chunks = (nm + per - 1) / per;
  for (int k = 0, off = 0; k < n_chunks; off += chunk_members(nm, n_chunks, k++)) {
    const int cnt = chunk_members(nm, n_chunks, k);
    DevCtx cc = c;
    cc.m0 = c.m0 + off;
    int grid = 0, per_cu = 0;
    int xcd_wg = 0;
    persist_shape(h, npb, cnt, &grid, &per_cu, fn, &xcd_wg);
    dfx_persist::launch_ring_poison(st, ring, h->pl.batch, h->pl.n_blocks, cc.m0, cnt, kPos);
    h->launches++;
    PersistArgs pa;
    pa.ring = ring; pa.give_up = persist_give_up_word(h); pa.n_steps = n_steps; pa.nm = cnt; pa.waves_per_member = h->persist_wpm; pa.spin_limit = persist_spin_limit(h); pa.xcd_wg = xcd_wg;
#ifdef DFX_PERSIST_TIMING
    pa.dbg = ((reverse ? getenv("DFX_TIMING_REVERSE") != nullptr : getenv("DFX_TIMING_REVERSE") == nullptr) && grid <= 8192) ? persist_dbg_buffer() : nullptr;
#endif
    void* args_f[] = {&cc, &pcf, &pa};
    void* args_r[] = {&cc, &pca, &pa};
    launch_persist(h, fn, st, reverse ? args_r : args_f, grid, per_cu * persist_wg_slots(fn));
  }
}
static void launch_fwd_persist(dfx_handle* h, const DevCtx& c, hipStream_t st, int nm, int n_steps) { launch_segment_persist(h, c, st, nm, n_steps, false); }

bool persist_adaptive_plan(dfx_handle* h) {
  h->persist_fwd = false;
  if (!persist_shape_ok(h) || h->groups.size() != 1 || h->pl.tab.s != 6) return false;
  const void* fn = dfx_persist::adaptive_fwd_kernel(h->pl.model, h->pl.contact);
  if (!fn) return false;
  h->persist_npb = 4;
  h->persist_wpm = (h->pl.n_slots + 63) / 64;
  h->persist_fwd_members = persist_members_that_fit(h, fn, 4);
  if (h->persist_fwd_members <= 0 || (h->pl.batch + h->persist_fwd_members - 1) / h->persist_fwd_members > 8) return false;
  const size_t B = h->pl.batch;
  if (h->d_ring.ensure((size_t)kPRing * B * h->pl.n_blocks * kPos) != hipSuccess || h->d_err3.ensure(3 * B * (size_t)h->persist_wpm) != hipSuccess) {
    (void)hipGetLastError();
    return false;
  }
  h->persist_fwd = true;
  return true;
}
void launch_adaptive_persist(dfx_handle* h, const DevCtx& c, hipStream_t st, int max_attempts, AdaptLoopArgs aa) {
  const void* fn = dfx_persist::adaptive_fwd_kernel(h->pl.model, h->pl.contact);
  const Dopri D = make_dopri();
  AdaptLoopCoef pc;
  memset(&pc, 0, sizeof(pc));
  for (int i = 0; i < 7; ++i) {
    pc.e[i] = D.e[i]; pc.ee[i] = D.ee[i]; pc.cm[i] = D.cm[i]; pc.cma[i] = D.cma[i]; pc.c[i] = D.c[i];
    for (int l = 0; l < 7; ++l) { pc.a[i][l] = D.a[i][l]; pc.aa[i][l] = D.aa[i][l]; }
  }
  const int nm = h->pl.batch, per = h->persist_fwd_members;
  const int n_chunks = (nm + per - 1) / per, even = (nm + n_chunks - 1) / n_chunks;
  aa.err = h->d_err3.p;
  (void)hipMemsetAsync(h->d_err3.p, 0xFF, sizeof(double) * 3 * (size_t)nm * h->persist_wpm, st);
  for (int off = 0; off < nm; off += even) {
    const int cnt = std::min(even, nm - off);
    DevCtx cc = c;
    cc.m0 = c.m0 + off;
    int grid = 0, per_cu = 0;
    int xcd_wg = 0;
    persist_shape(h, 4, cnt, &grid, &per_cu, fn, &xcd_wg);
    dfx_persist::launch_ring_poison(st, h->d_ring.p, h->pl.batch, h->pl.n_blocks, cc.m0, cnt, kPos);
    h->launches++;
    PersistArgs pa;
    pa.ring = h->d_ring.p; pa.give_up = persist_give_up_word(h); pa.n_steps = max_attempts; pa.nm = cnt; pa.waves_per_member = h->persist_wpm; pa.spin_limit = persist_spin_limit(h); pa.xcd_wg = xcd_wg;
#ifdef DFX_PERSIST_TIMING
    pa.dbg = nullptr;
#endif
    void* args[] = {&cc, &pc, &pa, &aa};
    launch_persist(h, fn, st, args, grid, per_cu * persist_wg_slots(fn));
  }
}
bool persist_plan_adj_dense(dfx_handle* h, const DevCtx& c) {
  h->persist_adj = false;
  if (!persist_common_ok(h, c)) return false;
  if (c.rps <= 1 || c.g_b || c.AD || !c.lam_pairs) return false;
  const void* fn = dfx_persist::adj_dense_kernel(h->pl.model, h->pl.contact, h->persist_npb);
  if (!fn) return false;
  h->persist_adj_members = persist_members_that_fit(h, fn, h->persist_npb);
  if (h->persist_adj_members <= 0 || (h->pl.batch + h->persist_adj_members - 1) / h->persist_adj_members > 8) return false;
  if (h->d_ring.ensure((size_t)kPRing * h->pl.batch * h->pl.n_blocks * kPos) != hipSuccess) { (void)hipGetLastError(); return false; }
  h->persist_adj = true;
  return true;
}
void launch_adj_dense_persist(dfx_handle* h, const DevCtx& c, hipStream_t st, int n_steps, DenseCtx dn) {
  const int npb = h->persist_npb, per = h->persist_adj_members, nm = h->pl.batch;
  const void* fn = dfx_persist::adj_dense_kernel(h->pl.model, h->pl.contact, npb);
  PersistAdjCoef pca;
  memset(&pca, 0, sizeof(pca));
  for (int i = 0; i < h->pl.tab.s && i < kPersistStages; ++i) {
    const AdjCoef ac = adj_coef(h->pl.tab, i);
    for (int jj = 0; jj <= kPersistStages; ++jj) { pca.col[i][jj] = ac.col[jj]; pca.cur[i][jj] = ac.cur[jj]; }
    pca.c[i] = ac.c_i;
  }
  const int n_chunks = (nm + per - 1) / per, even = (nm + n_chunks - 1) / n_chunks;
  for (int off = 0; off < nm; off += even) {
    const int cnt = std::min(even, nm - off);
    DevCtx cc = c;
    cc.m0 = c.m0 + off;
    int grid = 0, per_cu = 0;
    int xcd_wg = 0;
    persist_shape(h, npb, cnt, &grid, &per_cu, fn, &xcd_wg);
    dfx_persist::launch_ring_poison(st, h->d_ring.p, h->pl.batch, h->pl.n_blocks, cc.m0, cnt, kPos);
    h->launches++;
    PersistArgs pa;
    pa.ring = h->d_ring.p; pa.give_up = persist_give_up_word(h); pa.n_steps = n_steps; pa.nm = cnt; pa.waves_per_member = h->persist_wpm; pa.spin_limit = persist_spin_limit(h); pa.xcd_wg = xcd_wg;
#ifdef DFX_PERSIST_TIMING
    pa.dbg = nullptr;
#endif
    void* args[] = {&cc, &pca, &pa, &dn};
    launch_persist(h, fn, st, args, grid, per_cu * persist_wg_slots(fn));
  }
}
static void launch_adj_persist(dfx_handle* h, const DevCtx& c, hipStream_t st, int nm, int n_steps) { launch_segment_persist(h, c, st, nm, n_steps, true); }

static int fin(int i) { return i == 0 ? 0 : 1 + ((i - 1) & 1); }
static int fout(int i, int s) { return i == s - 1 ? 0 : 1 + (i & 1); }
static void launch_fwd_step_stage(dfx_handle* h, const DevCtx& c, hipStream_t st, dim3 grid, int i, int j) {
  const int s = h->pl.tab.s;
  if (c.rps > 1) launch_fwd(h, c, st, grid, i, j, -1 - i, -1 - (i + 1), -1, 0);
  else launch_fwd(h, c, st, grid, i, j, fin(i), fout(i, s), 0, (i == s - 1 && c.traj) ? 1 : 0);
}
static int adj_in_buf(const DevCtx& c, int i) { return c.rps > 1 ? -1 - i : (i == 0 ? -1 : i); }
int step_units(const dfx_handle* h, int kind) { return (kind == 0 ? h->pair_fwd : h->pair_adj) ? h->pl.tab.s / 2 : h->pl.tab.s; }
static void launch_fwd_unit(dfx_handle* h, const DevCtx& c, hipStream_t st, dim3 grid, int u, int j) {
  if (!h->pair_fwd) { launch_fwd_step_stage(h, c, st, grid, u, j); return; }
#ifdef DFX_EXPERIMENTAL
  const int s = h->pl.tab.s, i = 2 * u, nm = (int)grid.y;
  if (c.rps > 1) launch_fwd_pair(h, c, st, nm, i, j, -1 - i, -1 - (i + 1), -1 - (i + 2), -1, 0);
  else launch_fwd_pair(h, c, st, nm, i, j, u == 0 ? 0 : 1 + ((u - 1) & 1), -1, i + 2 == s ? 0 : 1 + (u & 1), 0, (i + 2 == s && c.traj) ? 1 : 0);
#endif
}
static void launch_adj_unit(dfx_handle* h, const DevCtx& c, hipStream_t st, dim3 grid, int u, int j) {
  const int s = h->pl.tab.s;
  if (!h->pair_adj) { const int i = s - 1 - u; launch_adj(h, c, st, grid, i, j, adj_in_buf(c, i), -1, 0); return; }
#ifdef DFX_EXPERIMENTAL
  launch_adj_pair(h, c, st, (int)grid.y, s - 1 - 2 * u, j);
#endif
}

bool use_fn_table(const dfx_handle* h) {
  const char* e = getenv("DFX_FN_TABLE");
  return h->pl.n_fns > 0 && !h->adaptive && h->d_fn_tab.p && !(e && e[0] == '0');
}
void launch_fn_table(dfx_handle* h, const DevCtx& c, hipStream_t st, int nm, int n_steps) {
  if (!c.fn_tab) return;
  StageTimes tms;
  for (int r = 0; r < kFnRows; ++r) tms.c[r] = r <= h->pl.tab.s ? h->pl.tab.c[r] : 0.0;
  const int total = n_steps * (h->pl.tab.s + 1) * h->pl.n_fns;
  hipLaunchKernelGGL(k_fn_table, dim3((total + 63) / 64, nm), dim3(64), 0, st, c, tms, n_steps, const_cast<double*>(c.fn_tab));
  h->launches++;
}

static void enqueue_segment(dfx_handle* h, const DevCtx& cbase, int gi, int n_steps, int kind) {
  const int s = h->pl.tab.s;
  const Group& g = h->groups[gi];
  const DevCtx c = group_ctx(h, cbase, gi);
  const dim3 grid = slot_grid(h, g);
  hipLaunchKernelGGL(k_tick, dim3(1), dim3(1), 0, g.stream, (const Seg*)h->d_segs.p, h->d_seg_idx.p + 2 + gi, kind == 0 ? 1 : -1, h->d_cur.p + gi);
  h->launches++;
  launch_fn_table(h, c, g.stream, g.nm, n_steps);
  if (kind == 0 && h->persist_fwd) launch_fwd_persist(h, c, g.stream, g.nm, n_steps);
  else if (kind == 0) {
    for (int j = 0; j < n_steps; ++j)
      for (int u = 0; u < step_units(h, 0); ++u) launch_fwd_unit(h, c, g.stream, grid, u, j);
  } else if (h->persist_adj) launch_adj_persist(h, c, g.stream, g.nm, n_steps);
  else if (c.AD || c.rps > 1) {
    for (int j = n_steps - 1; j >= 0; --j)
      for (int u = 0; u < step_units(h, 1); ++u) launch_adj_unit(h, c, g.stream, grid, u, j);
  } else if (!h->dual_chain) {
    for (int j = n_steps - 1; j >= 0; --j) {
      for (int i = 0; i < s - 1; ++i) launch_fwd(h, c, g.stream, grid, i, j, i == 0 ? -1 : i, i + 1, -1, 0);
      for (int i = s - 1; i >= 0; --i) launch_adj(h, c, g.stream, grid, i, j, i == 0 ? -1 : i, -1, 0);
    }
  } else {
    Group& gm = h->groups[gi];
    while ((int)gm.ev_a.size() < n_steps) {
      hipEvent_t a = nullptr, b = nullptr;
      (void)hipEventCreateWithFlags(&a, hipEventDisableTiming);
      (void)hipEventCreateWithFlags(&b, hipEventDisableTiming);
      gm.ev_a.push_back(a); gm.ev_b.push_back(b);
    }
    auto buf = [&](int j, int i) { return 1 + (j & 1) * (s - 1) + (i - 1); };
    (void)hipEventRecord(h->ev_fork2, g.stream);
    (void)hipStreamWaitEvent(g.stream2, h->ev_fork2, 0);
    for (int j = n_steps - 1; j >= 0; --j) {
      if (j + 2 <= n_steps - 1) (void)hipStreamWaitEvent(g.stream2, gm.ev_b[j + 2], 0);
      for (int i = 0; i < s - 1; ++i) launch_fwd(h, c, g.stream2, grid, i, j, i == 0 ? -1 : buf(j, i), buf(j, i + 1), -1, 0);
      (void)hipEventRecord(gm.ev_a[j], g.stream2);
      (void)hipStreamWaitEvent(g.stream, gm.ev_a[j], 0);
      for (int i = s - 1; i >= 0; --i) launch_adj(h, c, g.stream, grid, i, j, i == 0 ? -1 : buf(j, i), -1, 0);
      (void)hipEventRecord(gm.ev_b[j], g.stream);
    }
  }
}

bool solve_is_eager(const dfx_handle* h) {
  if (!h->use_graph) return true;
  if (const char* e = getenv("DFX_EAGER_STEPS")) return h->n_total <= atoll(e);
  const long long waves = (long long)h->pl.batch * ((h->pl.n_slots + 63) / 64);
  return waves >= 2048 || h->n_total <= 128;
}

void enqueue_interleaved(dfx_handle* h, const DevCtx& cbase, int n_steps, int kind, int seg_index) {
  const int ng = (int)h->groups.size();
  if (kind == 1 && !cbase.AD && cbase.rps == 1) {
    for (int gi = 0; gi < ng; ++gi) enqueue_segment(h, cbase, gi, n_steps, kind);
    return;
  }
  std::vector<DevCtx> cg(ng, cbase);
  for (int gi = 0; gi < ng; ++gi) {
    cg[gi] = group_ctx(h, cbase, gi);
    if (seg_index >= 0) hipLaunchKernelGGL(k_set_seg, dim3(1), dim3(1), 0, h->groups[gi].stream, (const Seg*)h->d_segs.p, seg_index, h->d_cur.p + gi);
    else hipLaunchKernelGGL(k_tick, dim3(1), dim3(1), 0, h->groups[gi].stream, (const Seg*)h->d_segs.p, h->d_seg_idx.p + 2 + gi, kind == 0 ? 1 : -1,
        h->d_cur.p + gi);
    h->launches++;
    launch_fn_table(h, cg[gi], h->groups[gi].stream, h->groups[gi].nm, n_steps);
  }
  if (kind == 0 && h->persist_fwd) {
    for (int gi = 0; gi < ng; ++gi) launch_fwd_persist(h, cg[gi], h->groups[gi].stream, h->groups[gi].nm, n_steps);
  } else if (kind == 0) {
    for (int j = 0; j < n_steps; ++j)
      for (int u = 0; u < step_units(h, 0); ++u)
        for (int gi = 0; gi < ng; ++gi)
          launch_fwd_unit(h, cg[gi], h->groups[gi].stream, slot_grid(h, h->groups[gi]), u, j);
  } else if (h->persist_adj) {
    Group& g0 = h->groups[0];
    for (int gi = 1; gi < ng; ++gi) {
      (void)hipEventRecord(h->groups[gi].done, h->groups[gi].stream);
      (void)hipStreamWaitEvent(g0.stream, h->groups[gi].done, 0);
    }
    launch_adj_persist(h, cg[0], g0.stream, ng > 1 ? h->pl.batch : g0.nm, n_steps);
    if (ng > 1) {
      (void)hipEventRecord(g0.done, g0.stream);
      for (int gi = 1; gi < ng; ++gi) (void)hipStreamWaitEvent(h->groups[gi].stream, g0.done, 0);
    }
  } else {
    for (int j = n_steps - 1; j >= 0; --j)
      for (int u = 0; u < step_units(h, 1); ++u)
        for (int gi = 0; gi < ng; ++gi)
          launch_adj_unit(h, cg[gi], h->groups[gi].stream, slot_grid(h, h->groups[gi]), u, j);
  }
}

bool seg_overlap_plan(dfx_handle* h, const DevCtx& c) {
  const char* e = getenv("DFX_SEG_OVERLAP");
  if ((e && e[0] == '0') || !h->segments || !h->persist_fwd || !h->persist_adj || h->groups.size() != 1 || h->pieces.size() < 2) return false;
  const int npb = h->persist_npb, nm = h->pl.batch;
  const void* ff = dfx_persist::fwd_kernel(h->pl.model, h->pl.contact, npb);
  const void* fr = dfx_persist::adj_kernel(h->pl.model, h->pl.contact, npb);
  if (h->persist_fwd_members < nm || h->persist_adj_members < nm) return false;
  int grid = 0, per_cu_f = 0, per_cu_r = 0, xf = 0, xr = 0;
  persist_shape(h, npb, nm, &grid, &per_cu_f, ff, &xf);
  persist_shape(h, npb, nm, &grid, &per_cu_r, fr, &xr);
  if (per_cu_f * persist_wg_slots(ff) + per_cu_r * persist_wg_slots(fr) > kPersistSlots) return false;
  const int of = persist_wg_per_cu(ff), orv = persist_wg_per_cu(fr), per_cu = std::max(per_cu_f, per_cu_r);
  if ((of && 2 * per_cu > of) || (orv && 2 * per_cu > orv)) return false;
  size_t steps = 0;
  for (const auto& pc : h->pieces) { size_t n = 0; for (int si = pc.first; si <= pc.last; ++si) n += h->segs[si].n_steps; steps = std::max(steps, n); }
  const size_t rec = (size_t)h->pl.n_blocks * kStep;
  const size_t want = (size_t)nm * (steps * h->pl.tab.s + 1) * rec;
  if (h->d_traj2.n < want) {
    size_t free_b = 0, total_b = 0;
    if (hipMemGetInfo(&free_b, &total_b) != hipSuccess) { (void)hipGetLastError(); return false; }
    if ((want - h->d_traj2.n) * sizeof(double) + total_b / 20 > free_b) return false;
  }
  if (h->d_traj2.ensure(want) != hipSuccess || h->d_ring2.ensure((size_t)kPRing * nm * h->pl.n_blocks * kPos) != hipSuccess ||
      (c.fn_tab && h->d_fn_tab2.ensure(h->d_fn_tab.n) != hipSuccess)) { (void)hipGetLastError(); return false; }
  for (int b = 0; b < 2; ++b) {
    if (!h->ev_rebuilt[b] && hipEventCreateWithFlags(&h->ev_rebuilt[b], hipEventDisableTiming) != hipSuccess) { (void)hipGetLastError(); return false; }
    if (!h->ev_reversed[b] && hipEventCreateWithFlags(&h->ev_reversed[b], hipEventDisableTiming) != hipSuccess) { (void)hipGetLastError(); return false; }
  }
  return true;
}
void enqueue_rerun_segment(dfx_handle* h, const DevCtx& cf, hipStream_t st, int seg_index) {
  const int n_steps = h->segs[seg_index].n_steps;
  hipLaunchKernelGGL(k_set_seg, dim3(1), dim3(1), 0, st, (const Seg*)h->d_segs.p, seg_index, const_cast<Seg*>(cf.cur));
  h->launches++;
  launch_fn_table(h, cf, st, h->pl.batch, n_steps);
  launch_segment_persist(h, cf, st, h->pl.batch, n_steps, false, h->d_ring2.p);
}

int run_segment(dfx_handle* h, const DevCtx& c, int gi, int n_steps, int kind) {
  if (!h->use_graph) { enqueue_segment(h, c, gi, n_steps, kind); return 0; }
  dfx_handle::GraphKey gk;
  memset(&gk, 0, sizeof(gk));
  memcpy(&gk.ctx, &c, sizeof(DevCtx));
  gk.ctx.n_timepoints = 0;
  gk.segs = h->d_segs.p; gk.seg_idx = h->d_seg_idx.p; gk.cur = h->d_cur.p;
  gk.pair_fwd = h->pair_fwd; gk.pair_adj = h->pair_adj; gk.pair_rows = h->pair_rows;
  if (!h->graph_ctx_valid || memcmp(&h->graph_key, &gk, sizeof(gk)) != 0) {
    drop_graphs(h);
    memcpy(&h->graph_key, &gk, sizeof(gk));
    h->graph_ctx_valid = true;
  }
  auto key = std::make_pair(n_steps, kind * kMaxGroups + gi);
  auto it = h->graphs.find(key);
  const int s = h->pl.tab.s;
  const long long per = 1 + (c.fn_tab ? 1 : 0) + (long long)n_steps * ((kind == 0 || c.AD || c.rps > 1) ? step_units(h, kind) : 2 * s - 1);
  hipStream_t st = h->groups[gi].stream;
  if (it == h->graphs.end()) {
    hipGraph_t graph = nullptr;
    hipGraphExec_t exec = nullptr;
    const long long before = h->launches;
    HIP_OK(hipStreamBeginCapture(st, hipStreamCaptureModeThreadLocal));
    enqueue_segment(h, c, gi, n_steps, kind);
    hipError_t ce = hipStreamEndCapture(st, &graph);
    h->launches = before;
    if (ce == hipSuccess) ce = hipGraphInstantiate(&exec, graph, nullptr, nullptr, 0);
    if (graph) (void)hipGraphDestroy(graph);
    if (ce != hipSuccess) { h->err = std::string("graph capture / instantiate: ") + hipGetErrorString(ce); return 2; }
    (void)hipGraphUpload(exec, st);
    it = h->graphs.emplace(key, exec).first;
  }
  HIP_OK(hipGraphLaunch(it->second, st));
  h->launches += per;
  return 0;
}

int fork_groups(dfx_handle* h) {
  HIP_OK(hipEventRecord(h->ev_fork, h->stream));
  for (auto& g : h->groups) if (g.stream != h->stream) HIP_OK(hipStreamWaitEvent(g.stream, h->ev_fork, 0));
  return 0;
}
int join_groups(dfx_handle* h) {
  for (auto& g : h->groups) {
    if (g.stream == h->stream) continue;
    HIP_OK(hipEventRecord(g.done, g.stream));
    HIP_OK(hipStreamWaitEvent(h->stream, g.done, 0));
  }
  return 0;
}
```

Before: 1.312 billion.

## Slim persistent kernel context, pre-offset member pointers, precompute per-stage coefficient rows

Replaces the large DevCtx kernel argument with a compact PersistCtx whose per-member pointers are pre-offset by m0 on the host. Coefficient tables are flattened into per-stage rows with masking baked in, so the inner loop does no index checks. Trajectory, function-table, AD and ring addresses are advanced incrementally and ring slots are chosen with a power-of-two mask, removing divisions and repeated address math from the hot stage loop. This aims to cut scalar and integer overhead and register pressure in the latency-bound persistent loops, at the cost of more host-side setup and a larger refactor that risks subtle indexing bugs.

After: 1.360 billion (median of 6 runs). 3.7% higher.

```diff
diff --git a/difflexmm_amd/csrc/dfx_persist.h b/difflexmm_amd/csrc/dfx_persist.h
--- a/difflexmm_amd/csrc/dfx_persist.h
+++ b/difflexmm_amd/csrc/dfx_persist.h
@@ -39,8 +39,8 @@
   double am, ac, kc, phi1, phi2, kap_safe, phi_min;
   int info, pslot;
 };
-template <int CONTACT>
-__device__ __forceinline__ void load_lig_res(const DevCtx& c, const MemberBases& B, int slot, LigRes& g) {
+template <int CONTACT, class Ctx >
+__device__ __forceinline__ void load_lig_res(const Ctx& c, const MemberBases& B, int slot, LigRes& g) {
   g.info = ldg<int>(c.slot_info, (u32)slot * 4);
   g.pslot = g.info < 0 ? slot : (g.info >> 1);
   g.sgn = (g.info & 1) ? 1.0 : -1.0;
@@ -65,6 +65,14 @@
     g.phi1 = ph.x; g.phi2 = ph.y;
   }
 }
+__device__ __forceinline__ int fresh_v(int x) { asm volatile("" : "+v"(x)); return x; }
+__device__ __forceinline__ MemberBases persist_bases(const PersistCtx& c, u32 um) {
+  MemberBases B{};
+  const u32 ps = um * (u32)c.n_slots;
+  B.p_r = c.p_r + (size_t)(ps * 2); B.p_phi = c.p_phi + (size_t)(ps * 2); B.p_l = c.p_l + (size_t)(ps * 2); B.p_k = c.p_k + (size_t)(ps * 4);
+  B.cst = c.cst + (size_t)(um * 16); B.l_dict = c.l_dict + (size_t)(um * 1024); B.p_lidx = c.p_lidx + (size_t)ps;
+  return B;
+}
 __device__ __forceinline__ bool ring_wait(const double* place, u32 byte_off, double (&r)[4], int t_ord, int* give_up, int limit) {
   for (int spins = 0;;) {
     ring_load(place, byte_off, r);
@@ -124,24 +132,24 @@
 #define DFX_PERSIST_OCC
 #endif
 template <int MODEL, int CONTACT, int NPB>
-__global__ __launch_bounds__(kPersistThreads) DFX_PERSIST_OCC void k_fwd_persist(DevCtx c, PersistCoef pc, PersistArgs pa) {
+__global__ __launch_bounds__(kPersistThreads) DFX_PERSIST_OCC void k_fwd_persist(PersistCtx c, PersistFwdTab pc, PersistArgs pa) {
   int ml, w;
   if (!persist_wave(pa, ml, w)) return;
-  const int m = c.m0 + ml;
   const LanePos lp = wave_lane_pos<NPB>(w, c.n_blocks);
   if (!lp.valid) return;
   const int slot = lp.slot, b = lp.b, k = lp.k, kd = k < 3 ? k : 2;
+  const u32 um = (u32)ml;
   const u32 nd = (u32)c.n_blocks * 3;
   const int s = c.s;
   const Seg sg = *c.cur;
-  const MemberBases B = member_bases(c, m);
+  const MemberBases B = persist_bases(c, um);
   LigRes g;
   load_lig_res<CONTACT>(c, B, slot, g);
   const int info = g.info, pslot = g.pslot;
   const int dof = b * 3 + kd;
   const u32 o_dof = (u32)dof * 8, o_rec = ((u32)b * kPos + kd) * 8, o_chunk = ((u32)b * kPos + 2 * (k & 1)) * 8;
-  const double damp = c.damping_uniform ? B.cst[6 + kd] : ldg<double>(c.damping + (size_t)((u32)m * nd), o_dof);
-  const double invm = ldg<double>(c.inv_m + (size_t)((u32)m * nd), o_dof);
+  const double damp = c.damping_uniform ? B.cst[6 + kd] : ldg<double>(c.damping + (size_t)(um * nd), o_dof);
+  const double invm = ldg<double>(c.inv_m + (size_t)(um * nd), o_dof);
   const int sidx = ldg<int>(c.block_special, (u32)b * 4);
   const bool constrained = k < 3 && sidx >= 0 && ((c.special[sidx >= 0 ? sidx : 0].con_mask >> k) & 1);
   double tf_coef[DFX_MAX_FNS];
@@ -150,11 +158,16 @@
     tf_coef[f] = (k < 3 && sidx >= 0 && f < c.n_fns) ? (constrained ? c.special[sidx].con_coef[k][f] : c.special[sidx].load_coef[k][f]) : 0.0;
   const bool recs = c.rps > 1;
   const long long n0 = sg.base_step;
+  const size_t blk = (size_t)((u32)c.n_blocks * (u32)kStep);
+  const size_t rec_step = (size_t)(u32)c.batch * blk;
+  double* const traj_m = c.traj ? c.traj + (size_t)um * blk : nullptr;
+  double* const POSm = c.POS + (size_t)(um * (u32)c.nbuf * (u32)c.n_blocks * (u32)kPos);
+  double* const VELm = c.VEL + (size_t)(um * (u32)c.nbuf * nd);
   double qn, vn;
   BlockRec<double> o;
   {
-    const double* P0 = pos_in(c, m, recs ? -1 : 0, n0);
-    const double* V0 = vel_in(c, m, recs ? -1 : 0, n0);
+    const double* P0 = recs ? traj_m + (size_t)((u32)n0 * (u32)c.rps) * rec_step : POSm;
+    const double* V0 = recs ? P0 + (size_t)((u32)c.n_blocks * (u32)kPos) : VELm;
     const double2 a0 = ldg<double2>(P0, (u32)b * kPos * 8), a1 = ldg<double2>(P0, (u32)b * kPos * 8 + 16);
     o.x = a0.x; o.y = a0.y; o.th = a1.x; o.sh = a1.y;
     qn = ldg<double>(P0, o_rec);
@@ -163,13 +176,22 @@
   double al[kPersistStages];
 #pragma unroll
   for (int l = 0; l < kPersistStages; ++l) al[l] = 0.0;
-  const size_t ring_stride = (size_t)c.batch * c.n_blocks * kPos;
-  const u32 r_own = ((u32)m * (u32)c.n_blocks + (u32)b) * (kPos * 8) + 16u * (u32)(k & 1);
-  const u32 r_par = ((u32)m * (u32)c.n_blocks + (u32)(pslot >> 2)) * (kPos * 8);
+  const size_t ring_stride = (size_t)((u32)c.batch * (u32)c.n_blocks * (u32)kPos);
+  const u32 r_own = (um * (u32)c.n_blocks + (u32)b) * (kPos * 8) + 16u * (u32)(k & 1);
+  const u32 r_par = (um * (u32)c.n_blocks + (u32)(pslot >> 2)) * (kPos * 8);
   if (k < 2) ring_store(pa.ring, r_own, k == 0 ? o.x : o.th, k == 0 ? o.y : o.sh);
   const int total = pa.n_steps * s;
   int t_ord = 0;
   double v_i = vn;
+  const int keep = recs ? 2 : (c.traj ? 1 : 0);
+  double* tr = keep ? traj_m + ((size_t)((u32)n0 * (u32)c.rps) + 1) * rec_step : nullptr;
+  const size_t rec_adv = recs ? rec_step : 0, rec_gap = recs ? (size_t)(u32)(c.rps - s) * rec_step : (keep ? rec_step : 0);
+  const u32 o_vrec = (u32)c.n_blocks * (kPos * 8) + o_dof;
+  const double* ft = c.fn_tab ? c.fn_tab + ((size_t)um * kMaxGraphSteps * kFnRows) * (DFX_MAX_FNS * kFnEntry) : nullptr;
+  const int ft_row = c.fn_tab ? DFX_MAX_FNS * kFnEntry : 0;
+  const u32 z_row = constrained ? (u32)(DFX_MAX_FNS * kFnEntry * 8) : 0u;
+  double* Am = c.AD ? c.AD + (size_t)um * c.ad_stride + (size_t)n0 * ((u32)(s - 1) * nd) : nullptr;
+  const double* place = pa.ring;
 #ifdef DFX_PERSIST_TIMING
   unsigned acc_t[6] = {0, 0, 0, 0, 0, 0};
   unsigned long long t_prev = tick();
@@ -178,35 +200,36 @@
   for (int j = 0; j < pa.n_steps; ++j) {
     const long long n = n0 + j;
     double h = sg.h;
-    if (c.t_steps) { const double* ts = steps_of(c, m); h = ts[n + 1] - ts[n]; }
-    double* Am = c.AD ? c.AD + (size_t)m * c.ad_stride + (size_t)n * ((u32)(s - 1) * nd) : nullptr;
+    if (c.t_steps) { const double* ts = c.t_steps + (size_t)um * (size_t)c.ts_stride; h = ts[n + 1] - ts[n]; }
 #pragma unroll 1
     for (int i = 0; i < s; ++i) {
       {
+        const double* row = pc.row[i];
+        double cv[kPersistStages - 1], cq[kPersistStages - 1];
+#pragma unroll
+        for (int l = 0; l < kPersistStages - 1; ++l) { cv[l] = row[l]; cq[l] = row[kPersistStages - 1 + l]; }
+        const double cv_i = row[10], cq_i = row[11], c_next = row[12];
         o.ch = half_cos(o.th, o.sh);
         double sv = 0.0, sq = 0.0, fload = 0.0;
 #pragma unroll
         for (int l = 0; l < kPersistStages - 1; ++l) {
-          const double a_l = l < i ? al[l] : 0.0;
-          sv += pc.cv[i][l] * a_l;
-          sq += pc.cq[i][l] * a_l;
+          sv += cv[l] * al[l];
+          sq += cq[l] * al[l];
         }
         double tv0[DFX_MAX_FNS], tv1[DFX_MAX_FNS];
 #pragma unroll
         for (int f = 0; f < DFX_MAX_FNS; ++f) { tv0[f] = 0.0; tv1[f] = 0.0; }
         if (k < 3 && sidx >= 0) {
-          const double* ft = fn_tab_row(c, m, j, constrained ? i + 1 : i);
-          const u32 z = lane_zero();
+          const u32 z = lane_zero() + z_row;
 #pragma unroll
           for (int f = 0; f < DFX_MAX_FNS; ++f)
             if (f < c.n_fns) { tv0[f] = fn_tab_get(ft, f, 0, z); if (constrained) tv1[f] = fn_tab_get(ft, f, 1, z); }
         }
         DFX_TICK(0)
-        const double* place = pa.ring + (size_t)(t_ord % kPRing) * ring_stride;
         double pr[4];
         if (!ring_wait(place, r_par, pr, t_ord, pa.give_up, pa.spin_limit)) return;
         DFX_TICK(1)
-        if (k < 2 && t_ord + kPAhead <= total) ring_poison(pa.ring + (size_t)((t_ord + kPAhead) % kPRing) * ring_stride, r_own);
+        if (k < 2 && t_ord + kPAhead <= total) ring_poison(pa.ring + (size_t)(((u32)t_ord + kPAhead) & (kPRing - 1)) * ring_stride, r_own);
         BlockRec<double> p;
         p.x = pr[0]; p.y = pr[1]; p.th = pr[2]; p.sh = pr[3];
         p.ch = half_cos(p.th, p.sh);
@@ -233,12 +256,12 @@
         double qnext = 0.0, vnext = 0.0;
         if (k < 3) {
           const double a = constrained ? 0.0 : (fload - dE - damp * v_i) * invm;
-          if (Am && i < s - 1) stg<double>(Am + (size_t)i * nd, o_dof, a);
-          sv += pc.cv[i][i] * a;
-          sq += pc.cq[i][i] * a;
+          if (Am && i < s - 1) stg<double>(Am, o_dof, a);
+          sv += cv_i * a;
+          sq += cq_i * a;
 #pragma unroll
           for (int l = 0; l < kPersistStages; ++l) al[l] = l == i ? a : al[l];
-          qnext = qn + h * (pc.c[i + 1] * vn + h * sq);
+          qnext = qn + h * (c_next * vn + h * sq);
           vnext = vn + h * sv;
           if (constrained) { qnext = q_pre; vnext = v_pre; }
         }
@@ -248,26 +271,31 @@
         fast_sincos(0.5 * th2, &sn, &cs);
         o.x = x0; o.y = y1; o.th = th2; o.sh = sn;
         ++t_ord;
+        place = pa.ring + (size_t)((u32)t_ord & (kPRing - 1)) * ring_stride;
         DFX_TICK(4)
         const bool last = i == s - 1;
-        if (k < 2) ring_store(pa.ring + (size_t)(t_ord % kPRing) * ring_stride, r_own, k == 0 ? x0 : th2, k == 0 ? y1 : sn);
+        if (k < 2) ring_store(const_cast<double*>(place), r_own, k == 0 ? x0 : th2, k == 0 ? y1 : sn);
         if (k < 3) {
           const double2 chunk = k == 0 ? make_double2(x0, y1) : make_double2(th2, sn);
-          if (recs || (last && c.traj)) {
-            double* tr = recs ? traj_rec(c, m, -2 - i, n) : traj_rec(c, m, -1, n + 1);
+          if (keep > (last ? 0 : 1)) {
             if (k < 2) stg<double2>(tr, o_chunk, chunk);
-            stg<double>(tr + (size_t)c.n_blocks * kPos, o_dof, vnext);
+            stg<double>(tr, o_vrec, vnext);
           }
-          if (last && !recs && j == pa.n_steps - 1) {
-            if (k < 2) stg<double2>(c.POS + (size_t)((u32)m * (u32)c.nbuf * (u32)c.n_blocks * kPos), o_chunk, chunk);
-            stg<double>(c.VEL + (size_t)((u32)m * (u32)c.nbuf * nd), o_dof, vnext);
+          if (last && keep < 2 && j == pa.n_steps - 1) {
+            if (k < 2) stg<double2>(POSm, o_chunk, chunk);
+            stg<double>(VELm, o_dof, vnext);
           }
         }
         v_i = vnext;
         if (last) { qn = qnext; vn = vnext; }
         DFX_TICK(5)
+        tr += rec_adv;
+        ft += ft_row;
+        if (Am && i < s - 1) Am += nd;
       }
     }
+    tr += rec_gap;
+    ft += (kFnRows - s) * ft_row;
   }
 #ifdef DFX_PERSIST_TIMING
   if (pa.dbg && (threadIdx.x & 63) == 0) {
@@ -287,59 +315,71 @@
 
 
 template <int MODEL, int CONTACT, int NPB, int DENSE>
-__device__ __forceinline__ void adj_persist_body(const DevCtx& c, const PersistAdjCoef& pc, const PersistArgs& pa, const DenseCtx& dn) {
+__device__ __forceinline__ void adj_persist_body(const PersistCtx& c, const PersistAdjTab& pc, const PersistArgs& pa, const DenseCtx& dn) {
   int ml, w;
   if (!persist_wave(pa, ml, w)) return;
-  const int m = c.m0 + ml;
   const LanePos lp = wave_lane_pos<NPB>(w, c.n_blocks);
   if (!lp.valid) return;
   const int slot = lp.slot, b = lp.b, k = lp.k, kd = k < 3 ? k : 2;
+  const u32 um = (u32)ml;
   const u32 nd = (u32)c.n_blocks * 3, nd6 = (u32)c.n_blocks * 6;
   const int s = c.s;
   const Seg sg = *c.cur;
   long long n_m = 0;
   int j_top = pa.n_steps - 1;
   if constexpr (DENSE) {
-    n_m = dn.n_acc[m];
+    n_m = dn.n_acc[c.m0 + ml];
     if (n_m - sg.base_step < (long long)j_top) j_top = (int)(n_m - sg.base_step);
     if (j_top < 0) return;
   }
-  const MemberBases B = member_bases(c, m);
+  const MemberBases B = persist_bases(c, um);
   LigRes g;
   load_lig_res<CONTACT>(c, B, slot, g);
   const int info = g.info, pslot = g.pslot;
   const int dof = b * 3 + kd;
   const u32 o_dof = (u32)dof * 8, o_b6 = ((u32)b * 6 + 2 * kd) * 8;
-  const double damp = c.damping_uniform ? B.cst[6 + kd] : ldg<double>(c.damping + (size_t)((u32)m * nd), o_dof);
-  const double invm = ldg<double>(c.inv_m + (size_t)((u32)m * nd), o_dof);
+  const double damp = c.damping_uniform ? B.cst[6 + kd] : ldg<double>(c.damping + (size_t)(um * nd), o_dof);
+  const double invm = ldg<double>(c.inv_m + (size_t)(um * nd), o_dof);
   const int sidx = ldg<int>(c.block_special, (u32)b * 4);
   const bool constrained = k < 3 && sidx >= 0 && ((c.special[sidx >= 0 ? sidx : 0].con_mask >> k) & 1);
   double tf_coef[DFX_MAX_FNS];
 #pragma unroll
   for (int f = 0; f < DFX_MAX_FNS; ++f)
     tf_coef[f] = (k < 3 && sidx >= 0 && f < c.n_fns) ? (constrained ? c.special[sidx].con_coef[k][f] : c.special[sidx].load_coef[k][f]) : 0.0;
-  double* LAMm = c.LAM + (size_t)((u32)m * nd6);
-  const u32 ms = (u32)m * (u32)c.n_slots;
+  double* LAMm = c.LAM + (size_t)(um * nd6);
+  const u32 ms = um * (u32)c.n_slots;
   double* grm = c.g_r + (size_t)(ms * 2);
   double* gpm = c.g_phi + (size_t)ms;
-  double* bmm = c.blk_m + (size_t)((u32)m * nd);
-  double* bcm = c.blk_c ? c.blk_c + (size_t)((u32)m * nd) : nullptr;
+  double* bmm = c.blk_m + (size_t)(um * nd);
+  double* bcm = c.blk_c ? c.blk_c + (size_t)(um * nd) : nullptr;
   __shared__ double2 s_yb[kPersistStages - 1][kPersistThreads];
   __shared__ double2 s_racc[kPersistThreads];
   __shared__ double s_acc[3][kPersistThreads];
   __shared__ double2 s_lam[kPersistThreads];
   const int tid = (int)threadIdx.x;
+#pragma unroll
+  for (int jj = 0; jj < kPersistStages - 1; ++jj) s_yb[jj][tid] = make_double2(0.0, 0.0);
   s_racc[tid] = ldg<double2>(grm, (u32)slot * 16);
   s_lam[tid] = ldg<double2>(LAMm, o_b6);
   s_acc[0][tid] = CONTACT == 1 ? ldg<double>(gpm, (u32)slot * 8) : 0.0;
   s_acc[1][tid] = ldg<double>(bmm, o_dof);
   s_acc[2][tid] = bcm ? ldg<double>(bcm, o_dof) : 0.0;
   bool phi_any = false;
-  const size_t ring_stride = (size_t)c.batch * c.n_blocks * kPos;
-  const u32 r_own = ((u32)m * (u32)c.n_blocks + (u32)b) * (kPos * 8) + 16u * (u32)(k & 1);
-  const u32 r_par = ((u32)m * (u32)c.n_blocks + (u32)(pslot >> 2)) * (kPos * 8);
+  double* const fn_gq = (c.fn_g && k < 3 && sidx >= 0) ? c.fn_g + (((size_t)um * c.n_special + sidx) * DFX_MAX_FNS) * DFX_FN_PARAMS : nullptr;
+  const size_t ring_stride = (size_t)((u32)c.batch * (u32)c.n_blocks * (u32)kPos);
+  const u32 r_own = (um * (u32)c.n_blocks + (u32)b) * (kPos * 8) + 16u * (u32)(k & 1);
+  const u32 r_par = (um * (u32)c.n_blocks + (u32)(pslot >> 2)) * (kPos * 8);
   const int total = DENSE ? (j_top + 1) * s - ((sg.base_step + j_top == n_m) ? s - 1 : 0) : pa.n_steps * s;
   int t_ord = 0;
+  const int i_top = (DENSE && sg.base_step + j_top == n_m) ? 0 : s - 1;
+  const size_t rec_step = (size_t)((u32)c.batch * ((u32)c.n_blocks * (u32)kStep));
+  const u32 o_vel = (u32)c.n_blocks * (kPos * 8) + o_dof;
+  const double* rec = c.traj + (size_t)((((u32)(sg.base_step + j_top) * (u32)c.rps + (u32)i_top) * (u32)c.batch + um)) * (size_t)((u32)c.n_blocks * (u32)kStep);
+  const size_t rec_gap = (size_t)(u32)(c.rps - s) * rec_step;
+  const double* ft = c.fn_tab ? c.fn_tab + (((size_t)um * kMaxGraphSteps + (u32)j_top) * kFnRows + (u32)i_top) * (DFX_MAX_FNS * kFnEntry) : nullptr;
+  const int ft_row = c.fn_tab ? DFX_MAX_FNS * kFnEntry : 0;
+  int win = (int)(((sg.base_step + j_top) * s + i_top) & 1);
+  const double* place = pa.ring;
 #ifdef DFX_PERSIST_TIMING
   unsigned acc_t[6] = {0, 0, 0, 0, 0, 0};
   unsigned long long t_prev = tick();
@@ -348,48 +388,56 @@
   for (int j = j_top; j >= 0; --j) {
     const long long n = sg.base_step + j;
     double h = sg.h, h_before = (sg.j0 + j) == 0 ? sg.h_prev : sg.h;
-    if (c.t_steps) { const double* ts = steps_of(c, m); h = ts[n + 1] - ts[n]; h_before = n > 0 ? ts[n] - ts[n - 1] : 0.0; }
+    if (c.t_steps) { const double* ts = c.t_steps + (size_t)um * (size_t)c.ts_stride; h = ts[n + 1] - ts[n]; h_before = n > 0 ? ts[n] - ts[n - 1] : 0.0; }
+    const bool first = !DENSE && (sg.j0 + j) == 0 && c.G;
+    double g0q = 0.0, g0v = 0.0;
+    if (first && k < 3 && !constrained) {
+      const double* G = c.G + ((size_t)sg.interval * c.batch + um) * (size_t)nd6;
+      g0q = G[b * 6 + k]; g0v = G[b * 6 + 3 + k];
+    }
 #pragma unroll 1
     for (int i = (DENSE && n == n_m) ? 0 : s - 1; i >= 0; --i) {
-      const int win = (int)((n * s + i) & 1);
-      const double* POSin = traj_rec(c, m, -1 - i, n);
+      const double* row = pc.row[i];
+      double cf[kPersistStages - 1], cu[kPersistStages - 1];
+#pragma unroll
+      for (int jj = 0; jj < kPersistStages - 1; ++jj) { cf[jj] = row[jj]; cu[jj] = row[kPersistStages - 1 + jj]; }
+      const double col_s = row[10], cur_s = row[11], col_i = row[12];
+      const double* POSin = rec;
       const double2 o0 = ldg<double2>(POSin, (u32)b * (kPos * 8)), o1 = ldg<double2>(POSin, (u32)b * (kPos * 8) + 16);
       const double2 q0 = ldg<double2>(POSin, (u32)(pslot >> 2) * (kPos * 8)), q1 = ldg<double2>(POSin, (u32)(pslot >> 2) * (kPos * 8) + 16);
-      const double v_i = ldg<double>(POSin + (size_t)c.n_blocks * kPos, o_dof);
+      const double v_i = ldg<double>(POSin, o_vel);
       double sq = 0.0, sv = 0.0, sqc = 0.0, svc = 0.0;
 #pragma unroll
       for (int jj = 1; jj < kPersistStages; ++jj) {
-        const bool on = jj > i && jj < s && !(DENSE && n == n_m);
-        const double2 y = on ? s_yb[jj - 1][tid] : make_double2(0.0, 0.0);
-        const double cf = i > 0 ? pc.col[i][jj] : 1.0;
-        sq += cf * y.x;
-        sv += cf * y.y;
-        sqc += pc.cur[i][jj] * y.x;
-        svc += pc.cur[i][jj] * y.y;
-      }
+        const double2 y = s_yb[jj - 1][tid];
+        sq += cf[jj - 1] * y.x;
+        sv += cf[jj - 1] * y.y;
+        sqc += cu[jj - 1] * y.x;
+        svc += cu[jj - 1] * y.y;
+      }
+      asm volatile("" : "+v"(sq), "+v"(sv), "+v"(sqc), "+v"(svc));
       double tv0[DFX_MAX_FNS];
 #pragma unroll
       for (int f = 0; f < DFX_MAX_FNS; ++f) tv0[f] = 0.0;
       if (k < 3 && sidx >= 0 && !constrained) {
-        const double* ft = fn_tab_row(c, m, j, i);
         const u32 z = lane_zero();
 #pragma unroll
         for (int f = 0; f < DFX_MAX_FNS; ++f) if (f < c.n_fns) tv0[f] = fn_tab_get(ft, f, 0, z);
       }
-      const double col_s = pc.col[i][s], cur_s = pc.cur[i][s], col_i = pc.col[i][i];
       const double2 lam = s_lam[tid];
       const double lq = lam.x, lv = lam.y;
       double w_d = (h * (cur_s * lv + svc)) * invm;
       double e_own_q = 0.0, e_nxt_v = 0.0, gs_q = 0.0, gs_v = 0.0;
       if constexpr (DENSE) {
         if (!constrained) {
+          const int m = c.m0 + ml;
           const int* op = dn.out_ptr + (size_t)m * dn.stride;
           const int lo = op[n], hi = op[n + 1], plo = n > 0 ? op[n - 1] : lo;
           const double* dwm = dn.dw + (size_t)m * dn.n_out * 8;
           const u32 o_g = ((u32)b * 6 + kd) * 8;
           double e_own_v = 0.0;
           for (int kk = lo; kk < hi; ++kk) {
-            const double* Gk = c.G + ((size_t)kk * c.batch + m) * (size_t)nd6;
+            const double* Gk = c.G + ((size_t)kk * c.batch + um) * (size_t)nd6;
             const double gq = ldg<double>(Gk, o_g), gv = ldg<double>(Gk, o_g + 24);
             const double* wt = dwm + (size_t)kk * 8;
             e_own_q += wt[i] * gq; e_own_v += wt[i] * gv;
@@ -400,7 +448,7 @@
           if (i <= 1) {
             double e6q = 0.0, e6v = 0.0, e5v = 0.0;
             for (int kk = plo; kk < lo; ++kk) {
-              const double* Gk = c.G + ((size_t)kk * c.batch + m) * (size_t)nd6;
+              const double* Gk = c.G + ((size_t)kk * c.batch + um) * (size_t)nd6;
               const double gq = ldg<double>(Gk, o_g), gv = ldg<double>(Gk, o_g + 24);
               const double* wt = dwm + (size_t)kk * 8;
               e6q += wt[6] * gq; e6v += wt[6] * gv;
@@ -411,7 +459,7 @@
           }
           if (i == 0 && n == 0)
             for (int kk = 0; kk < lo; ++kk) {
-              const double* Gk = c.G + ((size_t)kk * c.batch + m) * (size_t)nd6;
+              const double* Gk = c.G + ((size_t)kk * c.batch + um) * (size_t)nd6;
               gs_q += ldg<double>(Gk, o_g); gs_v += ldg<double>(Gk, o_g + 24);
             }
           w_d += e_own_v * invm;
@@ -421,13 +469,13 @@
       double wp[4];
       DFX_TICK(0)
       if (t_ord == 0) {
-        const double* Win = c.W + (size_t)(((u32)m * 2 + (u32)win) * nd);
+        const double* Win = c.W + (size_t)((um * 2 + (u32)win) * nd);
         const u32 pb = (u32)(pslot >> 2) * 24;
         const double2 wxy = ldg<double2>(Win, pb);
         wp[0] = wxy.x; wp[1] = wxy.y; wp[2] = ldg<double>(Win, pb + 16);
-      } else if (!ring_wait(pa.ring + (size_t)(t_ord % kPRing) * ring_stride, r_par, wp, t_ord, pa.give_up, pa.spin_limit)) return;
+      } else if (!ring_wait(place, r_par, wp, t_ord, pa.give_up, pa.spin_limit)) return;
       DFX_TICK(1)
-      if (k < 2 && t_ord + kPAhead < total) ring_poison(pa.ring + (size_t)((t_ord + kPAhead) % kPRing) * ring_stride, r_own);
+      if (k < 2 && t_ord + kPAhead < total) ring_poison(pa.ring + (size_t)(((u32)t_ord + kPAhead) & (kPRing - 1)) * ring_stride, r_own);
       BlockRec<double> o, p;
       o.x = o0.x; o.y = o0.y; o.th = o1.x; o.sh = o1.y; o.ch = half_cos(o.th, o.sh);
       p.x = q0.x; p.y = q0.y; p.th = q1.x; p.sh = q1.y; p.ch = half_cos(p.th, p.sh);
@@ -458,14 +506,14 @@
         double fload = 0.0;
 #pragma unroll
         for (int f = 0; f < DFX_MAX_FNS; ++f) if (!constrained) fload += tf_coef[f] * tv0[f];
-        if (c.fn_g && sidx >= 0) {
-          const double* ft = fn_tab_row(c, m, j, i);
+        double* const fq = fn_gq;
+        if (fresh_v(fq != nullptr)) {
 #pragma unroll
           for (int f = 0; f < DFX_MAX_FNS; ++f) {
             const double coef = f < c.n_fns ? (constrained ? -hw * tf_coef[f] : w_d * tf_coef[f]) : 0.0;
             if (coef != 0.0) {
               const u32 z = lane_zero();
-              double* q = c.fn_g + (((size_t)m * c.n_special + sidx) * DFX_MAX_FNS + f) * DFX_FN_PARAMS;
+              double* q = fq + f * DFX_FN_PARAMS;
               for (int kk = 0; kk < DFX_FN_PARAMS; ++kk) acc_add(q + kk, coef * fn_tab_get(ft, f, 2 + kk, z));
             }
           }
@@ -487,11 +535,7 @@
         } else {
           double nlq = lq + (ybq + sq), nlv = lv + (ybv + sv);
           if constexpr (DENSE) { nlq += gs_q; nlv += gs_v; }
-          const bool first = !DENSE && (sg.j0 + j) == 0;
-          if (first && c.G && !constrained) {
-            const double* G = c.G + ((size_t)sg.interval * c.batch + m) * (size_t)nd6;
-            nlq += G[b * 6 + k]; nlv += G[b * 6 + 3 + k];
-          }
+          if (first) { nlq += g0q; nlv += g0v; }
           if (constrained) { nlq = 0.0; nlv = 0.0; }
           s_lam[tid] = make_double2(nlq, nlv);
           kv = h_before * col_s * nlv;
@@ -501,13 +545,19 @@
       }
       DFX_TICK(3)
       ++t_ord;
+      place = pa.ring + (size_t)((u32)t_ord & (kPRing - 1)) * ring_stride;
       if (t_ord < total) {
         const double w1 = blk_bcast<NPB, 1>(w_next, k), w2 = blk_bcast<NPB, 2>(w_next, k);
-        if (k < 2) ring_store(pa.ring + (size_t)(t_ord % kPRing) * ring_stride, r_own, k == 0 ? w_next : w2, k == 0 ? w1 : 0.0);
+        if (k < 2) ring_store(const_cast<double*>(place), r_own, k == 0 ? w_next : w2, k == 0 ? w1 : 0.0);
       } else if (k < 3) {
-        stg<double>(c.W + (size_t)(((u32)m * 2 + (u32)(win ^ 1)) * nd), o_dof, w_next);
-      }
+        stg<double>(c.W + (size_t)((um * 2 + (u32)(win ^ 1)) * nd), o_dof, w_next);
+      }
+      rec -= rec_step;
+      ft -= ft_row;
+      win ^= 1;
     }
+    rec -= rec_gap;
+    ft -= (kFnRows - s) * ft_row;
   }
 #ifdef DFX_PERSIST_TIMING
   if (pa.dbg && (threadIdx.x & 63) == 0) {
@@ -525,7 +575,7 @@
 }
 
 template <int MODEL, int CONTACT, int NPB>
-__global__ __launch_bounds__(kPersistThreads) __attribute__((amdgpu_waves_per_eu(3))) void k_adj_persist(DevCtx c, PersistAdjCoef pc, PersistArgs pa) {
+__global__ __launch_bounds__(kPersistThreads) __attribute__((amdgpu_waves_per_eu(3))) void k_adj_persist(PersistCtx c, PersistAdjTab pc, PersistArgs pa) {
   adj_persist_body<MODEL, CONTACT, NPB, 0>(c, pc, pa, DenseCtx{});
 }
 
diff --git a/difflexmm_amd/csrc/dfx_persist_api.h b/difflexmm_amd/csrc/dfx_persist_api.h
--- a/difflexmm_amd/csrc/dfx_persist_api.h
+++ b/difflexmm_amd/csrc/dfx_persist_api.h
@@ -28,10 +28,30 @@
 };
 
 
-struct PersistAdjCoef {
-  double col[kPersistStages][kPersistStages + 1];
-  double cur[kPersistStages][kPersistStages + 1];
-  double c[kPersistStages];
+constexpr int kAdjRow = 16;
+struct PersistAdjTab { double row[kPersistStages][kAdjRow]; };
+struct PersistFwdTab { double row[kPersistStages][kAdjRow]; };
+static_assert((kPRing & (kPRing - 1)) == 0, "the ring place of a stage ordinal is taken with a mask");
+
+struct PersistCtx {
+  int n_blocks, n_slots, n_fns, batch, s, rps, n_special, m0;
+  int k_uniform, damping_uniform, l_dict_on, nbuf;
+  const int32_t* slot_info;
+  const int32_t* block_special;
+  const dfx_special* special;
+  const double *p_r, *p_l, *p_k, *p_phi, *l_dict, *cst, *inv_m, *damping;
+  const uint8_t* p_lidx;
+  const double* fn_tab;
+  const dfx::Seg* cur;
+  const double* t_steps;
+  long long ts_stride;
+  double* traj;
+  double *POS, *VEL, *AD;
+  long long ad_stride;
+  double *LAM, *W;
+  const double* G;
+  double *g_r, *g_phi, *blk_m, *blk_c, *fn_g;
+  int* touch;
 };
 
 const void* fwd_kernel(int model, int contact, int npb);
diff --git a/difflexmm_amd/csrc/dfx_persist_dense.h b/difflexmm_amd/csrc/dfx_persist_dense.h
--- a/difflexmm_amd/csrc/dfx_persist_dense.h
+++ b/difflexmm_amd/csrc/dfx_persist_dense.h
@@ -299,7 +299,7 @@
 }
 
 template <int MODEL, int CONTACT, int NPB>
-__global__ __launch_bounds__(kPersistThreads) DFX_DENSE_OCC void k_adj_dense_loop(DevCtx c, PersistAdjCoef pc, PersistArgs pa,
+__global__ __launch_bounds__(kPersistThreads) DFX_DENSE_OCC void k_adj_dense_loop(PersistCtx c, PersistAdjTab pc, PersistArgs pa,
                                                                                                            DenseCtx dn) {
   adj_persist_body<MODEL, CONTACT, NPB, 1>(c, pc, pa, dn);
 }
diff --git a/difflexmm_amd/csrc/engine_launch.hip b/difflexmm_amd/csrc/engine_launch.hip
--- a/difflexmm_amd/csrc/engine_launch.hip
+++ b/difflexmm_amd/csrc/engine_launch.hip
@@ -441,18 +441,64 @@
   fl.push_back({ev, st, need});
   h->launches++;
 }
+static PersistAdjTab persist_adj_tab(const Tableau& T) {
+  PersistAdjTab t;
+  memset(&t, 0, sizeof(t));
+  const int s = T.s;
+  for (int i = 0; i < s && i < kPersistStages; ++i) {
+    const AdjCoef ac = adj_coef(T, i);
+    for (int jj = 1; jj < kPersistStages; ++jj) {
+      const bool on = jj > i && jj < s;
+      t.row[i][jj - 1] = on ? (i > 0 ? ac.col[jj] : 1.0) : 0.0;
+      t.row[i][kPersistStages - 1 + jj - 1] = on ? ac.cur[jj] : 0.0;
+    }
+    t.row[i][10] = ac.col[s]; t.row[i][11] = ac.cur[s]; t.row[i][12] = ac.col[i];
+  }
+  return t;
+}
+static PersistFwdTab persist_fwd_tab(const Tableau& T) {
+  const PersistCoef pc = persist_coef(T);
+  PersistFwdTab t;
+  memset(&t, 0, sizeof(t));
+  for (int i = 0; i < T.s && i < kPersistStages; ++i) {
+    for (int l = 0; l < kPersistStages - 1 && l < i; ++l) { t.row[i][l] = pc.cv[i][l]; t.row[i][kPersistStages - 1 + l] = pc.cq[i][l]; }
+    t.row[i][10] = pc.cv[i][i]; t.row[i][11] = pc.cq[i][i]; t.row[i][12] = pc.c[i + 1];
+  }
+  return t;
+}
+template <class P> static P* persist_at(P* p, size_t elems) { return p ? p + elems : p; }
+static PersistCtx persist_ctx(const DevCtx& cc) {
+  PersistCtx p;
+  memset(&p, 0, sizeof(p));
+  const size_t m0 = (size_t)cc.m0, nd = (size_t)cc.n_blocks * 3, ns = (size_t)cc.n_slots;
+  p.n_blocks = cc.n_blocks; p.n_slots = cc.n_slots; p.n_fns = cc.n_fns; p.batch = cc.batch; p.s = cc.s; p.rps = cc.rps;
+  p.n_special = cc.n_special; p.m0 = cc.m0;
+  p.k_uniform = cc.k_uniform; p.damping_uniform = cc.damping_uniform; p.l_dict_on = cc.l_dict_on;
+  p.slot_info = cc.slot_info; p.block_special = cc.block_special; p.special = cc.special;
+  p.p_r = persist_at(cc.p_r, m0 * ns * 2); p.p_l = persist_at(cc.p_l, m0 * ns * 2); p.p_k = persist_at(cc.p_k, m0 * ns * 4);
+  p.p_phi = persist_at(cc.p_phi, m0 * ns * 2); p.l_dict = persist_at(cc.l_dict, m0 * 1024); p.cst = persist_at(cc.cst, m0 * 16);
+  p.p_lidx = persist_at(cc.p_lidx, m0 * ns);
+  p.inv_m = persist_at(cc.inv_m, m0 * nd); p.damping = persist_at(cc.damping, m0 * nd);
+  p.fn_tab = persist_at(cc.fn_tab, m0 * kMaxGraphSteps * kFnRows * (DFX_MAX_FNS * kFnEntry));
+  p.cur = cc.cur;
+  p.t_steps = persist_at(cc.t_steps, m0 * (size_t)cc.ts_stride); p.ts_stride = cc.ts_stride;
+  p.traj = persist_at(cc.traj, m0 * (size_t)cc.n_blocks * kStep);
+  p.nbuf = cc.nbuf; p.ad_stride = cc.ad_stride;
+  p.POS = persist_at(cc.POS, m0 * cc.nbuf * (size_t)cc.n_blocks * kPos); p.VEL = persist_at(cc.VEL, m0 * cc.nbuf * nd);
+  p.AD = persist_at(cc.AD, m0 * (size_t)cc.ad_stride);
+  p.LAM = persist_at(cc.LAM, m0 * nd * 2); p.W = persist_at(cc.W, m0 * 2 * nd); p.G = persist_at(cc.G, m0 * nd * 2);
+  p.g_r = persist_at(cc.g_r, m0 * ns * 2); p.g_phi = persist_at(cc.g_phi, m0 * ns);
+  p.blk_m = persist_at(cc.blk_m, m0 * nd); p.blk_c = persist_at(cc.blk_c, m0 * nd);
+  p.fn_g = persist_at(cc.fn_g, m0 * (size_t)cc.n_special * DFX_MAX_FNS * DFX_FN_PARAMS);
+  p.touch = cc.touch;
+  return p;
+}
 static void launch_segment_persist(dfx_handle* h, const DevCtx& c, hipStream_t st, int nm, int n_steps, bool reverse, double* ring = nullptr) {
   if (!ring) ring = h->d_ring.p;
   const int npb = h->persist_npb, per = reverse ? h->persist_adj_members : h->persist_fwd_members;
   const void* fn = reverse ? dfx_persist::adj_kernel(h->pl.model, h->pl.contact, npb) : dfx_persist::fwd_kernel(h->pl.model, h->pl.contact, npb);
-  PersistCoef pcf = persist_coef(h->pl.tab);
-  PersistAdjCoef pca;
-  memset(&pca, 0, sizeof(pca));
-  for (int i = 0; i < h->pl.tab.s && i < kPersistStages; ++i) {
-    const AdjCoef ac = adj_coef(h->pl.tab, i);
-    for (int jj = 0; jj <= kPersistStages; ++jj) { pca.col[i][jj] = ac.col[jj]; pca.cur[i][jj] = ac.cur[jj]; }
-    pca.c[i] = ac.c_i;
-  }
+  PersistFwdTab pcf = persist_fwd_tab(h->pl.tab);
+  PersistAdjTab pca = persist_adj_tab(h->pl.tab);
   const int n_chunks = (nm + per - 1) / per;
   for (int k = 0, off = 0; k < n_chunks; off += chunk_members(nm, n_chunks, k++)) {
     const int cnt = chunk_members(nm, n_chunks, k);
@@ -464,12 +510,14 @@
     dfx_persist::launch_ring_poison(st, ring, h->pl.batch, h->pl.n_blocks, cc.m0, cnt, kPos);
     h->launches++;
     PersistArgs pa;
-    pa.ring = ring; pa.give_up = persist_give_up_word(h); pa.n_steps = n_steps; pa.nm = cnt; pa.waves_per_member = h->persist_wpm; pa.spin_limit = persist_spin_limit(h); pa.xcd_wg = xcd_wg;
+    pa.give_up = persist_give_up_word(h); pa.n_steps = n_steps; pa.nm = cnt; pa.waves_per_member = h->persist_wpm; pa.spin_limit = persist_spin_limit(h); pa.xcd_wg = xcd_wg;
 #ifdef DFX_PERSIST_TIMING
     pa.dbg = ((reverse ? getenv("DFX_TIMING_REVERSE") != nullptr : getenv("DFX_TIMING_REVERSE") == nullptr) && grid <= 8192) ? persist_dbg_buffer() : nullptr;
 #endif
-    void* args_f[] = {&cc, &pcf, &pa};
-    void* args_r[] = {&cc, &pca, &pa};
+    pa.ring = ring + (size_t)cc.m0 * h->pl.n_blocks * kPos;
+    PersistCtx pcx = persist_ctx(cc);
+    void* args_f[] = {&pcx, &pcf, &pa};
+    void* args_r[] = {&pcx, &pca, &pa};
     launch_persist(h, fn, st, reverse ? args_r : args_f, grid, per_cu * persist_wg_slots(fn));
   }
 }
@@ -538,13 +586,7 @@
 void launch_adj_dense_persist(dfx_handle* h, const DevCtx& c, hipStream_t st, int n_steps, DenseCtx dn) {
   const int npb = h->persist_npb, per = h->persist_adj_members, nm = h->pl.batch;
   const void* fn = dfx_persist::adj_dense_kernel(h->pl.model, h->pl.contact, npb);
-  PersistAdjCoef pca;
-  memset(&pca, 0, sizeof(pca));
-  for (int i = 0; i < h->pl.tab.s && i < kPersistStages; ++i) {
-    const AdjCoef ac = adj_coef(h->pl.tab, i);
-    for (int jj = 0; jj <= kPersistStages; ++jj) { pca.col[i][jj] = ac.col[jj]; pca.cur[i][jj] = ac.cur[jj]; }
-    pca.c[i] = ac.c_i;
-  }
+  PersistAdjTab pca = persist_adj_tab(h->pl.tab);
   const int n_chunks = (nm + per - 1) / per, even = (nm + n_chunks - 1) / n_chunks;
   for (int off = 0; off < nm; off += even) {
     const int cnt = std::min(even, nm - off);
@@ -556,11 +598,13 @@
     dfx_persist::launch_ring_poison(st, h->d_ring.p, h->pl.batch, h->pl.n_blocks, cc.m0, cnt, kPos);
     h->launches++;
     PersistArgs pa;
-    pa.ring = h->d_ring.p; pa.give_up = persist_give_up_word(h); pa.n_steps = n_steps; pa.nm = cnt; pa.waves_per_member = h->persist_wpm; pa.spin_limit = persist_spin_limit(h); pa.xcd_wg = xcd_wg;
+    pa.ring = h->d_ring.p + (size_t)cc.m0 * h->pl.n_blocks * kPos;
+    pa.give_up = persist_give_up_word(h); pa.n_steps = n_steps; pa.nm = cnt; pa.waves_per_member = h->persist_wpm; pa.spin_limit = persist_spin_limit(h); pa.xcd_wg = xcd_wg;
 #ifdef DFX_PERSIST_TIMING
     pa.dbg = nullptr;
 #endif
-    void* args[] = {&cc, &pca, &pa, &dn};
+    PersistCtx pcx = persist_ctx(cc);
+    void* args[] = {&pcx, &pca, &pa, &dn};
     launch_persist(h, fn, st, args, grid, per_cu * persist_wg_slots(fn));
   }
 }
```
